# nateraw/pytorchvideo-accelerate

Hardware: AMD Instinct MI355X
Metric: clips/sec (whole node) SlowFast-R50 32x2x224 at 1/2/4/8 MI355X; step-time p50 (higher is better)
Workload: dtype bf16; 1 GPU; model=SlowFast-R50 32x2x224, global_batch=160, per_gpu_batch=160, grad_accum=1, seq_len=32, parallelism=dp1, backend=none, comm=none, forced_sync=False, grad_dtype=fp32, classes=400, hip_graph=False, deterministic=True

## Files before the change

### csrc/kernels/bn_eltwise.hip

```cpp
#include "common.h"
#include <algorithm>

PVA_NS_BEGIN

namespace {

constexpr int NT = 256;

#define ROW_VEC_SETUP(CH)                                  \
  const int vecs = (CH) >> 3;                              \
  const int rpi = NT / vecs;                               \
  const int lr = threadIdx.x / vecs;                       \
  const int c = (threadIdx.x - lr * vecs) << 3;            \
  if (lr >= rpi) return;

__global__ void bn_finalize_kernel(const float* __restrict__ part, int tiles, int C, int64_t count,
                                   const float* __restrict__ gamma, const float* __restrict__ beta,
                                   float* __restrict__ run_mean, float* __restrict__ run_var,
                                   int64_t* __restrict__ nbt, float momentum, float eps,
                                   float* __restrict__ save_mean, float* __restrict__ save_rstd,
                                   float* __restrict__ scale, float* __restrict__ shift) {
  const int c = blockIdx.x;
  double s = 0.0, q = 0.0;
  for (int t = threadIdx.x; t < tiles; t += NT) {
// ... 383 lines not shown
    }
    if constexpr (Y1) {
      float b[8];
      unpack8(*reinterpret_cast<const uint4*>(y1 + m * C + c), b);
#pragma unroll
      for (int e = 0; e < 8; ++e) o[e] = A1[e] * dz[e] + B1[e] * b[e] + C1[e];
      *reinterpret_cast<uint4*>(dy1 + m * C + c) = pack8(o);
    }
    if constexpr (DZ) {
      uint16_t* d = dzout + m * lddz + c;
      if (dz_accum) {
        float q[8];
        unpack8(*reinterpret_cast<const uint4*>(d), q);
#pragma unroll
        for (int e = 0; e < 8; ++e) dz[e] += q[e];
      }
      *reinterpret_cast<uint4*>(d) = pack8(dz);
    }
  }
}

__global__ void stem_pool_fwd_kernel(const uint16_t* __restrict__ y, const float* __restrict__ scale,
                                     const float* __restrict__ shift, uint16_t* __restrict__ out,
                                     uint8_t* __restrict__ arg, uint16_t* __restrict__ ymax, int NT_, int H, int W,
                                     int Ho, int Wo, int C, int ldo) {
  ROW_VEC_SETUP(C);
  float sc[8], sh[8];
#pragma unroll
  for (int e = 0; e < 8; ++e) { sc[e] = scale[c + e]; sh[e] = shift[c + e]; }
  const int Q = NT_ * Ho * Wo;
  for (int q = blockIdx.x * rpi + lr; q < Q; q += gridDim.x * rpi) {
    const int wo = q % Wo;
    const int r = q / Wo;
    const int ho = r % Ho;
    const int nt = r / Ho;
    uint4 v[9];
#pragma unroll
    for (int dh = 0; dh < 3; ++dh)
#pragma unroll
      for (int dw = 0; dw < 3; ++dw) {
        const int h = min(max(ho * 2 - 1 + dh, 0), H - 1), w = min(max(wo * 2 - 1 + dw, 0), W - 1);
        v[dh * 3 + dw] = *reinterpret_cast<const uint4*>(y + (((int64_t)nt * H + h) * W + w) * C + c);
      }
    float best[8], yb[8];
    uint32_t bi[8];
#pragma unroll
    for (int e = 0; e < 8; ++e) { best[e] = -INFINITY; bi[e] = 0; yb[e] = 0.f; }
#pragma unroll
    for (int k = 0; k < 9; ++k) {
      const int h = ho * 2 - 1 + k / 3, w = wo * 2 - 1 + k % 3;
      if ((unsigned)h >= (unsigned)H || (unsigned)w >= (unsigned)W) continue;
      float f[8];
      unpack8(v[k], f);
#pragma unroll
      for (int e = 0; e < 8; ++e) {
        const float a = fmaxf(f[e] * sc[e] + sh[e], 0.f);
        if (a > best[e]) { best[e] = a; bi[e] = (uint32_t)k; yb[e] = f[e]; }
      }
    }
    const int64_t o = (int64_t)q * C + c;
    *reinterpret_cast<uint4*>(out + (int64_t)q * ldo + c) = pack8(best);
    uint2 pk;
    pk.x = bi[0] | (bi[1] << 8) | (bi[2] << 16) | (bi[3] << 24);
    pk.y = bi[4] | (bi[5] << 8) | (bi[6] << 16) | (bi[7] << 24);
    *reinterpret_cast<uint2*>(arg + o) = pk;
    if (ymax) *reinterpret_cast<uint4*>(ymax + o) = pack8(yb);
  }
}

__global__ void stem_pool_bwd_kernel(const uint16_t* __restrict__ dout, int ldd, const uint8_t* __restrict__ arg,
                                     uint16_t* __restrict__ dact, int NT_, int H, int W, int Ho, int Wo, int C) {
  const int vecs = C >> 3;
  const int64_t total = (int64_t)NT_ * H * W * vecs;
  for (int64_t i = blockIdx.x * (int64_t)NT + threadIdx.x; i < total; i += (int64_t)gridDim.x * NT) {
    int64_t r = i;
    const int cv = r % vecs; r /= vecs;
    const int w = r % W; r /= W;
    const int h = r % H; r /= H;
    const int64_t nt = r;
    const int c = cv << 3;
    float acc[8];
#pragma unroll
    for (int e = 0; e < 8; ++e) acc[e] = 0.f;
    const int ho_lo = (h) / 2, ho_hi = min(Ho - 1, (h + 1) / 2);
    const int wo_lo = (w) / 2, wo_hi = min(Wo - 1, (w + 1) / 2);
    for (int ho = ho_lo; ho <= ho_hi; ++ho) {
      const int dh = h - (ho * 2 - 1);
      if (dh < 0 || dh > 2) continue;
      for (int wo = wo_lo; wo <= wo_hi; ++wo) {
        const int dw = w - (wo * 2 - 1);
        if (dw < 0 || dw > 2) continue;
        const int64_t o = (nt * Ho + ho) * Wo + wo;
        const uint2 pk = *reinterpret_cast<const uint2*>(arg + o * C + c);
        float g[8];
        unpack8(*reinterpret_cast<const uint4*>(dout + o * ldd + c), g);
        const uint8_t want = (uint8_t)(dh * 3 + dw);
        uint8_t bi[8] = {(uint8_t)(pk.x), (uint8_t)(pk.x >> 8), (uint8_t)(pk.x >> 16), (uint8_t)(pk.x >> 24),
                         (uint8_t)(pk.y), (uint8_t)(pk.y >> 8), (uint8_t)(pk.y >> 16), (uint8_t)(pk.y >> 24)};
#pragma unroll
        for (int e = 0; e < 8; ++e) if (bi[e] == want) acc[e] += g[e];
      }
    }
    *reinterpret_cast<uint4*>(dact + ((nt * H + h) * W + w) * C + c) = pack8(acc);
  }
}

__global__ void stem_pool_bn_apply_kernel(const uint16_t* __restrict__ dout, int ldd, const uint8_t* __restrict__ arg,
                                          const uint16_t* __restrict__ y, const float* __restrict__ ms,
                                          const float* __restrict__ mh, const float* __restrict__ coef,
                                          uint16_t* __restrict__ dy, int NT_, int H, int W, int Ho, int Wo, int C) {
  ROW_VEC_SETUP(C);
  float A[8], B[8], Cc[8], MS[8], MH[8];
#pragma unroll
  for (int e = 0; e < 8; ++e) {
    A[e] = coef[c + e]; B[e] = coef[C + c + e]; Cc[e] = coef[2 * C + c + e];
    MS[e] = ms[c + e]; MH[e] = mh[c + e];
  }
  const int Q = NT_ * Ho * Wo;
  for (int q = blockIdx.x * rpi + lr; q < Q; q += gridDim.x * rpi) {
    const int wo = q % Wo;
    const int r = q / Wo;
    const int ho = r % Ho;
    const int nt = r / Ho;
    uint2 ag[2][2];
    float g[2][2][8];
#pragma unroll
    for (int i = 0; i < 2; ++i)
#pragma unroll
      for (int j = 0; j < 2; ++j) {
        const bool ok = ho + i < Ho && wo + j < Wo;
        const int64_t o = ((int64_t)nt * Ho + min(ho + i, Ho - 1)) * Wo + min(wo + j, Wo - 1);
        ag[i][j] = *reinterpret_cast<const uint2*>(arg + o * C + c);
        if (!ok) ag[i][j] = make_uint2(0xffffffffu, 0xffffffffu);
        unpack8(*reinterpret_cast<const uint4*>(dout + o * ldd + c), g[i][j]);
      }
#pragma unroll
    for (int a = 0; a < 2; ++a) {
      const int h = 2 * ho + a;
      if (h >= H) continue;
#pragma unroll
      for (int b = 0; b < 2; ++b) {
        const int w = 2 * wo + b;
        if (w >= W) continue;
        const int64_t m = ((int64_t)nt * H + h) * W + w;
        float yv[8], acc[8];
        unpack8(*reinterpret_cast<const uint4*>(y + m * C + c), yv);
#pragma unroll
        for (int e = 0; e < 8; ++e) acc[e] = 0.f;
#pragma unroll
        for (int i = 0; i <= a; ++i)
#pragma unroll
          for (int j = 0; j <= b; ++j) {
            const uint32_t want = (uint32_t)((i ? 0 : a + 1) * 3 + (j ? 0 : b + 1));
            const uint2 pk = ag[i][j];
#pragma unroll
            for (int e = 0; e < 8; ++e) {
              const uint32_t bi = ((e < 4 ? pk.x : pk.y) >> (8 * (e & 3))) & 255u;
              acc[e] += bi == want ? g[i][j][e] : 0.f;
            }
          }
        float o8[8];
#pragma unroll
        for (int e = 0; e < 8; ++e) {
          const float dz = (yv[e] * MS[e] + MH[e]) > 0.f ? acc[e] : 0.f;
          o8[e] = A[e] * dz + B[e] * yv[e] + Cc[e];
        }
        *reinterpret_cast<uint4*>(dy + m * C + c) = pack8(o8);
      }
    }
  }
}

__global__ void avgpool_global_part_kernel(const uint16_t* __restrict__ x, int vol, int C, int S,
                                           float* __restrict__ part) {
  const int n = blockIdx.x / S, sp = blockIdx.x % S;
  const int vecs = C >> 3;
  const int rpi = NT / vecs;
  const int lr = threadIdx.x / vecs;
  const int c = (threadIdx.x - lr * vecs) << 3;
  const int per = (vol + S - 1) / S;
  const int p0 = sp * per, p1 = min(vol, p0 + per);
  float s[8];
#pragma unroll
  for (int e = 0; e < 8; ++e) s[e] = 0.f;
  if (lr < rpi) {
    const uint16_t* base = x + (int64_t)n * vol * C + c;
    int p = p0 + lr;
    for (; p + 3 * rpi < p1; p += 4 * rpi) {
      uint4 q[4];
#pragma unroll
      for (int k = 0; k < 4; ++k) q[k] = *reinterpret_cast<const uint4*>(base + (int64_t)(p + k * rpi) * C);
#pragma unroll
      for (int k = 0; k < 4; ++k) {
        float f[8];
        unpack8(q[k], f);
#pragma unroll
        for (int e = 0; e < 8; ++e) s[e] += f[e];
      }
    }
    for (; p < p1; p += rpi) {
      float f[8];
      unpack8(*reinterpret_cast<const uint4*>(base + (int64_t)p * C), f);
#pragma unroll
      for (int e = 0; e < 8; ++e) s[e] += f[e];
    }
  }
  __shared__ float red[NT * 8];
#pragma unroll
  for (int e = 0; e < 8; ++e) red[threadIdx.x * 8 + e] = s[e];
  __syncthreads();
  for (int i = threadIdx.x; i < C; i += NT) {
    const int v = i >> 3, e = i & 7;
    float t = 0.f;
    for (int k = 0; k < rpi; ++k) t += red[(k * vecs + v) * 8 + e];
    part[((int64_t)n * S + sp) * C + i] = t;
  }
}

__global__ void avgpool_global_final_kernel(const float* __restrict__ part, int S, int C, float inv,
                                            float* __restrict__ out, int ldo, int coff, int N) {
  const int i = blockIdx.x * NT + threadIdx.x;
  if (i >= N * C) return;
  const int n = i / C, c = i % C;
  float t = 0.f;
  for (int k = 0; k < S; ++k) t += part[((int64_t)n * S + k) * C + c];
  out[(int64_t)n * ldo + coff + c] = t * inv;
}

__global__ void avgpool_global_bwd_kernel(const float* __restrict__ dout, int ldo, int coff, int vol, int C,
                                          float inv, uint16_t* __restrict__ dx, int64_t M) {
  ROW_VEC_SETUP(C);
  for (int64_t m = (int64_t)blockIdx.x * rpi + lr; m < M; m += (int64_t)gridDim.x * rpi) {
    const int64_t n = m / vol;
    const float4* src = reinterpret_cast<const float4*>(dout + n * ldo + coff + c);
    const float4 u = src[0], v = src[1];
    float f[8] = {u.x * inv, u.y * inv, u.z * inv, u.w * inv, v.x * inv, v.y * inv, v.z * inv, v.w * inv};
    *reinterpret_cast<uint4*>(dx + m * C + c) = pack8(f);
  }
}

__global__ void avgpool_fwd_kernel(const uint16_t* __restrict__ x, int T, int H, int W, int C, int kt, int kh, int kw,
                                   float* __restrict__ out, int ldo, int coff, int N) {
  const int To = T - kt + 1, Ho = H - kh + 1, Wo = W - kw + 1;
  const int P = To * Ho * Wo;
  const int cg = (C + 63) / 64;
  int b = blockIdx.x;
  const int g = b % cg; b /= cg;
  const int pos = b % P;
  const int n = b / P;
  const int to = pos / (Ho * Wo), ho = (pos / Wo) % Ho, wo = pos % Wo;
  const int lane = threadIdx.x & 63, w = threadIdx.x >> 6;
  const int c = g * 64 + lane;
  const int vol = kt * kh * kw;
  float s = 0.f;
  if (c < C) {
    for (int i = w; i < vol; i += 4) {
      const int a = i / (kh * kw), r = i % (kh * kw), bb = r / kw, d = r % kw;
      s += e2f(x[((((int64_t)n * T + to + a) * H + ho + bb) * W + wo + d) * C + c]);
    }
  }
  __shared__ float red[4][64];
  red[w][lane] = s;
  __syncthreads();
  if (w == 0 && c < C) {
    const float t = red[0][lane] + red[1][lane] + red[2][lane] + red[3][lane];
    out[((int64_t)n * P + pos) * ldo + coff + c] = t / (float)vol;
  }
}

__global__ void avgpool_bwd_kernel(const float* __restrict__ dout, int ldo, int coff, int T, int H, int W, int C,
                                   int kt, int kh, int kw, uint16_t* __restrict__ dx, int N) {
  const int To = T - kt + 1, Ho = H - kh + 1, Wo = W - kw + 1;
  const int64_t total = (int64_t)N * T * H * W * C;
  const float inv = 1.f / (float)(kt * kh * kw);
  for (int64_t i = blockIdx.x * (int64_t)NT + threadIdx.x; i < total; i += (int64_t)gridDim.x * NT) {
    int64_t r = i;
    const int c = r % C; r /= C;
    const int w = r % W; r /= W;
    const int h = r % H; r /= H;
    const int t = r % T; r /= T;
    const int n = (int)r;
    float s = 0.f;
    for (int to = max(0, t - kt + 1); to <= min(To - 1, t); ++to)
      for (int ho = max(0, h - kh + 1); ho <= min(Ho - 1, h); ++ho)
        for (int wo = max(0, w - kw + 1); wo <= min(Wo - 1, w); ++wo)
          s += dout[(((int64_t)n * To + to) * Ho + ho) * Wo * ldo + (int64_t)wo * ldo + coff + c];
    dx[i] = f2e(s * inv);
  }
}

int grid_for(int64_t work) {
  int64_t b = (work + NT - 1) / NT;
  if (b > 8192) b = 8192;
  if (b < 1) b = 1;
  return (int)b;
}

int grid_rows(int64_t M, int C) {
  const int rpi = NT / (C / 8);
  int64_t b = (M + (int64_t)rpi * 4 - 1) / ((int64_t)rpi * 4);
  if (b > 16384) b = 16384;
  if (b < 1) b = 1;
  return (int)b;
}

}

int bn_fin_ranges(int tiles) { return std::min(256, std::max(1, (tiles + FIN_TILES_PER_BLOCK - 1) / FIN_TILES_PER_BLOCK)); }

void bn_finalize_launch(const float* part, int tiles, int C, int64_t count, const float* gamma, const float* beta,
                        float* rm, float* rv, int64_t* nbt, float momentum, float eps, float* smean, float* srstd,
                        float* scale, float* shift, hipStream_t s, double* scratch, unsigned* ctr) {
  if (scratch && ctr) {
    hipLaunchKernelGGL(bn_finalize2_kernel, dim3((C + 63) / 64, bn_fin_ranges(tiles)), dim3(NT), 0, s, part, tiles, C,
                       count, gamma, beta, rm, rv, nbt, momentum, eps, smean, srstd, scale, shift, scratch, ctr);
    return;
  }
  hipLaunchKernelGGL(bn_finalize_kernel, dim3(C), dim3(NT), 0, s, part, tiles, C, count, gamma, beta, rm, rv, nbt,
                     momentum, eps, smean, srstd, scale, shift);
}
// ... 158 lines not shown
```

### csrc/kernels/common.h

```cpp
#pragma once
#include <hip/hip_runtime.h>
#include <stdint.h>

#ifndef PVA_F16
#define PVA_F16 0
#endif
#if PVA_F16
#define PVA_NS pva_f16
typedef _Float16 e16s_t;
#define PVA_MFMA16 __builtin_amdgcn_mfma_f32_16x16x32_f16
#else
#define PVA_NS pva_bf16
typedef __bf16 e16s_t;
#define PVA_MFMA16 __builtin_amdgcn_mfma_f32_16x16x32_bf16
#endif
#define PVA_NS_BEGIN namespace PVA_NS {
#define PVA_NS_END }

typedef uint16_t e16_t;
typedef __attribute__((ext_vector_type(8))) e16s_t ev8_t;
typedef __attribute__((ext_vector_type(4))) float f32x4_t;
typedef __attribute__((ext_vector_type(4))) short s16x4_t;
typedef __attribute__((ext_vector_type(8))) short s16x8_t;
typedef __attribute__((ext_vector_type(2))) float f32x2_t;
typedef __attribute__((ext_vector_type(2))) e16s_t ev2_t;
typedef __attribute__((ext_vector_type(2))) short s16x2_t;

#define PVA_WAVE 64
#define PVA_NXCD 8

#if PVA_F16
__device__ __forceinline__ float e2f(e16_t v) { return (float)__builtin_bit_cast(_Float16, v); }
__device__ __forceinline__ float lo2f(uint32_t w) { return e2f((e16_t)(w & 0xffffu)); }
__device__ __forceinline__ float hi2f(uint32_t w) { return e2f((e16_t)(w >> 16)); }
#else
__device__ __forceinline__ float e2f(e16_t v) { return __uint_as_float(((uint32_t)v) << 16); }
__device__ __forceinline__ float lo2f(uint32_t w) { return __uint_as_float(w << 16); }
__device__ __forceinline__ float hi2f(uint32_t w) { return __uint_as_float(w & 0xffff0000u); }
#endif

__device__ __forceinline__ e16_t f2e(float f) {
  e16s_t b = (e16s_t)f;
  return __builtin_bit_cast(e16_t, b);
}

__device__ __forceinline__ uint32_t cvt_pk_e16(float a, float b) {
  return __builtin_bit_cast(uint32_t, __builtin_convertvector((f32x2_t){a, b}, ev2_t));
}

__device__ __forceinline__ uint32_t pack2(float a, float b) { return cvt_pk_e16(a, b); }

__device__ __forceinline__ void unpack8(const uint4& v, float* f) {
  f[0] = lo2f(v.x); f[1] = hi2f(v.x);
  f[2] = lo2f(v.y); f[3] = hi2f(v.y);
  f[4] = lo2f(v.z); f[5] = hi2f(v.z);
  f[6] = lo2f(v.w); f[7] = hi2f(v.w);
}

__device__ __forceinline__ uint4 pack8(const float* f) {
  return make_uint4(pack2(f[0], f[1]), pack2(f[2], f[3]), pack2(f[4], f[5]), pack2(f[6], f[7]));
}


__device__ __forceinline__ uint4 pack8_fast(const float* f) {
  return make_uint4(cvt_pk_e16(f[0], f[1]), cvt_pk_e16(f[2], f[3]), cvt_pk_e16(f[4], f[5]), cvt_pk_e16(f[6], f[7]));
}

__device__ __forceinline__ uint32_t relu_e16x2(uint32_t w) {
  return __builtin_bit_cast(uint32_t, __builtin_elementwise_max(__builtin_bit_cast(s16x2_t, w), (s16x2_t){0, 0}));
}

__device__ __forceinline__ uint4 relu_e16x8(const uint4& v) {
  return make_uint4(relu_e16x2(v.x), relu_e16x2(v.y), relu_e16x2(v.z), relu_e16x2(v.w));
}

__device__ __forceinline__ uint32_t max_e16x2(uint32_t w, uint32_t floor) {
  return __builtin_bit_cast(uint32_t, __builtin_elementwise_max(__builtin_bit_cast(s16x2_t, w),
                                                                __builtin_bit_cast(s16x2_t, floor)));
}

__device__ __forceinline__ void unpack4(const uint2& v, float* f) {
  f[0] = lo2f(v.x); f[1] = hi2f(v.x);
  f[2] = lo2f(v.y); f[3] = hi2f(v.y);
}

__device__ __forceinline__ uint2 pack4(const float* f) {
  return make_uint2(pack2(f[0], f[1]), pack2(f[2], f[3]));
}

__device__ __forceinline__ int xcd_remap(int orig, int nwg) {
  if (nwg < PVA_NXCD * 2) return orig;
  const int q = nwg / PVA_NXCD, r = nwg % PVA_NXCD;
  const int xcd = orig % PVA_NXCD;
  return (xcd < r ? xcd * (q + 1) : r * (q + 1) + (xcd - r) * q) + orig / PVA_NXCD;
}


template <int CTRL>
__device__ __forceinline__ float dpp_f(float v) {
  return __builtin_bit_cast(float, __builtin_amdgcn_update_dpp(0, __builtin_bit_cast(int, v), CTRL, 0xf, 0xf, false));
}

__device__ __forceinline__ float sum16(float v) {
  v += dpp_f<0xB1>(v);
  v += dpp_f<0x4E>(v);
  v += dpp_f<0x141>(v);
  v += dpp_f<0x140>(v);
  return v;
}

template <int G>
__device__ __forceinline__ float sum_lanes(float v) {
  static_assert(G == 1 || G == 2 || G == 4 || G == 8 || G == 16, "DPP lane groups stay inside a 16-lane row");
  if constexpr (G >= 2) v += dpp_f<0xB1>(v);
  if constexpr (G >= 4) v += dpp_f<0x4E>(v);
  if constexpr (G >= 8) v += dpp_f<0x141>(v);
  if constexpr (G >= 16) v += dpp_f<0x140>(v);
  return v;
}

__device__ __forceinline__ float swap_sum16(float v) {
  const auto r = __builtin_amdgcn_permlane16_swap(__float_as_uint(v), __float_as_uint(v), true, false);
  const unsigned a = r[0], b = r[1];
  return __uint_as_float(a) + __uint_as_float(b);
}
__device__ __forceinline__ float swap_sum32(float v) {
  const auto r = __builtin_amdgcn_permlane32_swap(__float_as_uint(v), __float_as_uint(v), true, false);
  const unsigned a = r[0], b = r[1];
  return __uint_as_float(a) + __uint_as_float(b);
}

template <int S>
__device__ __forceinline__ float wave_sum_stride_c(float v) {
  static_assert(S >= 1 && S <= 64 && (S & (S - 1)) == 0, "stride");
  if constexpr (S <= 1) v += dpp_f<0xB1>(v);
  if constexpr (S <= 2) v += dpp_f<0x4E>(v);
  if constexpr (S <= 4) v += dpp_f<0x124>(v);
  if constexpr (S <= 8) v += dpp_f<0x128>(v);
  if constexpr (S <= 16) v = swap_sum16(v);
  if constexpr (S <= 32) v = swap_sum32(v);
  return v;
}

__device__ __forceinline__ float wave_sum(float v) { return swap_sum32(swap_sum16(sum16(v))); }

__device__ __forceinline__ unsigned swap_partner16(unsigned v) {
  const auto r = __builtin_amdgcn_permlane16_swap(v, v, true, false);
  const unsigned a = r[0], b = r[1];
  return a ^ b ^ v;
}

__device__ __forceinline__ float wave_sum_stride(float v, int S) {
  switch (S) {
    case 1: return wave_sum_stride_c<1>(v);
    case 2: return wave_sum_stride_c<2>(v);
    case 4: return wave_sum_stride_c<4>(v);
    case 8: return wave_sum_stride_c<8>(v);
    case 16: return wave_sum_stride_c<16>(v);
    case 32: return wave_sum_stride_c<32>(v);
    default:
      for (int off = S; off < 64; off <<= 1) v += __shfl_xor(v, off, 64);
      return v;
  }
}

__device__ __forceinline__ float sum_hi4(float v) {
  v += __shfl_xor(v, 16, 64);
  v += __shfl_xor(v, 32, 64);
  return v;
}
```

### csrc/kernels/launchers.h

```cpp
void conv_igemm_launch(const ConvParams& p, int chunk, hipStream_t stream, int cfg);
int conv_cfg_bm(int cfg, int N);
int conv_igemm_ut_legal(const ConvParams& p, int chunk, int bk);
int conv_direct_legal(const ConvParams& p, int chunk);
int conv_pw_legal(const ConvParams& p, int chunk);
int conv_halo_legal(const ConvParams& p, int chunk);
int conv_halo_epi_ok(const ConvParams& p);
int conv_halo64p_legal(const ConvParams& p, int chunk);
void conv_igemm_set_ut(int mode);
int conv_igemm_m_tiles(int M, int N);
int conv_igemm_m_tiles_k(int M, int N, int K, int Cg);
void conv_igemm_set_bk(int bk);
void conv_wgrad_launch(const WgradParams& p, int chunk, hipStream_t stream);
void conv_wgrad_tile(int Cout, int K, int variant, int* bmw, int* bnw);
int wgrad_rt_legal(int Cout, int Cin, int ldd, int ldx, int chunk, int dy_affine);
int wgrad_narrow_legal(int Cout, int Cin, int K);
int wgrad_halo_legal(const WgradParams& p);
int wgrad_box_legal(const WgradParams& p);
void wgrad_box_reduce_launch(const float* slab, float* tmp, float* grad, int splits, int Cout, int taps, int Cin,
                             int Cin_real, float scale, float beta, hipStream_t st);
int wgrad_box_reduce_groups(int splits);
void wgrad_reduce_launch(float* accbuf, float* grad, int splits, int Cout, int taps, int Cin, int Cin_real,
                         float scale, float beta, int slab, hipStream_t stream);
void bn_finalize_launch(const float* part, int tiles, int C, int64_t count, const float* gamma, const float* beta,
                        float* rm, float* rv, int64_t* nbt, float momentum, float eps, float* smean, float* srstd,
                        float* scale, float* shift, hipStream_t s, double* scratch, unsigned* ctr);
int bn_fin_ranges(int tiles);
void bn_eval_affine_launch(int C, const float* gamma, const float* beta, const float* rm, const float* rv, float eps,
                           float* scale, float* shift, hipStream_t s);
void bn_act_launch(const uint16_t* y, int ldy, uint16_t* out, int ldo, const float* scale, const float* shift,
                   int relu, int64_t M, int C, hipStream_t s);
void res_out_launch(const uint16_t* yc, const float* sc, const float* hc, const uint16_t* y1, const float* s1,
                    const float* h1, const uint16_t* x, int ldx, uint16_t* out, int ldo, uint8_t* mask, int64_t M,
                    int C, hipStream_t s);
int bn_bwd_reduce_blocks(int64_t M, int C, int* rows_per_block);
void bn_bwd_reduce_launch(const uint16_t* g, int ldg, int mask_mode, const void* mo, int ldm, const float* ms,
                          const float* mh, const uint16_t* y0, const float* mean0, const float* rstd0,
                          const uint16_t* y1, const float* mean1, const float* rstd1, int64_t M, int C, int blocks,
                          int rows_per_block, float* part, uint16_t* dzout, int lddz, hipStream_t s);
void bn_bwd_finalize_launch(const float* part, int blocks, int C, int64_t count, int which, const float* gamma,
                            const float* mean, const float* rstd, float* dgamma, float* dbeta, float beta_acc,
                            float* coef, hipStream_t s, double* scratch, unsigned* ctr);
void bn_bwd_apply_launch(const uint16_t* g, int ldg, int mask_mode, const void* mo, int ldm, const float* ms,
                         const float* mh, const uint16_t* y0, const float* coef0, uint16_t* dy0, const uint16_t* y1,
                         const float* coef1, uint16_t* dy1, uint16_t* dzout, int lddz, int dz_accum, int64_t M, int C,
                         hipStream_t s);
void stem_pool_fwd_launch(const uint16_t* y, const float* scale, const float* shift, uint16_t* out, uint8_t* arg,
                          uint16_t* ymax, int NT_, int H, int W, int Ho, int Wo, int C, int ldo, hipStream_t s);
void stem_pool_bn_apply_launch(const uint16_t* dout, int ldd, const uint8_t* arg, const uint16_t* y, const float* ms,
                               const float* mh, const float* coef, uint16_t* dy, int NT_, int H, int W, int Ho, int Wo,
                               int C, hipStream_t s);
int avgpool_global_splits(int N, int vol);
void stem_pool_bwd_launch(const uint16_t* dout, int ldd, const uint8_t* arg, uint16_t* dact, int NT_, int H, int W,
                          int Ho, int Wo, int C, hipStream_t s);
void avgpool_fwd_launch(const uint16_t* x, int N, int T, int H, int W, int C, int kt, int kh, int kw, float* out,
                        int ldo, int coff, float* scratch, hipStream_t s);
void avgpool_bwd_launch(const float* dout, int ldo, int coff, int N, int T, int H, int W, int C, int kt, int kh,
                        int kw, uint16_t* dx, hipStream_t s);
void sgd_momentum_launch(float* p, const float* g, float* buf, int64_t n, const float* lr, float momentum, float wd,
                         float gscale, int first, int* found_inf, const int* skip_flag, hipStream_t s);
void nonfinite_check_launch(const float* g, int64_t n, float gscale, int* flag, hipStream_t s);
void pack_weights_launch(const float* master, uint16_t* fwd, uint16_t* dgr, const void* descs, int ntensors,
                         hipStream_t s);
int pack_desc_size();
void video_preprocess_launch(const uint8_t* frames, const int* desc, const int* tidx, int B, int T, int S,
                             const float* mean, const float* std_, uint16_t* out, int s2d, hipStream_t s,
                             const int* slow_of = nullptr, uint16_t* slow_out = nullptr, int Ts = 0);
int stem_tiles(int Ho, int Wo, int N);
void stem_s2d_launch(int mode, const uint16_t* x, const uint16_t* w, uint16_t* y, float* stats, const uint16_t* dy,
                     float* dw, int N, int T, int Hs, int Ws, int Cout, int kt, hipStream_t s, float* slab = nullptr);
bool stem_s2d_supported(int Cout, int kt);
void stem_wgrad_convert_launch(float* acc, float* grad, int Cout, int kt, float beta, hipStream_t s);
void stem_pack_launch(const float* w, uint16_t* out, int Cout, int kt, hipStream_t s);
void synth_frames_launch(uint8_t* out, int64_t n, uint32_t seed, hipStream_t s);

void bnfold_fwd_stats_launch(const uint16_t* Wf, const float* Ga, const float* sslab, int splits, int C, int c,
                             int64_t count, float* T, float* s_out, const float* gamma, const float* beta, float* rm,
                             float* rv, int64_t* nbt, float momentum, float eps, float* smean, float* srstd,
                             float* scale, float* shift, hipStream_t st);
void bnfold_bwd_launch(const float* part, int tiles, const uint16_t* Wf, const uint16_t* Wd, const float* G,
                       const float* T, const float* s, int C, int c, int64_t count, const float* gamma,
                       const float* mean, const float* rstd, float* dgamma, float* dbeta, float* dW, float beta_acc,
                       float* coef, uint16_t* W1t, uint16_t* W2, float* bias, hipStream_t st);
void head_forward_launch(const float* feat, int N, int P, int C, const float* W, const float* b, int K, float p_drop,
                         uint64_t seed, const uint64_t* seedp, float* xm, float* logits, hipStream_t s);
void head_seed_advance_launch(uint64_t* seed, hipStream_t s);
void head_ce_launch(const float* logits, const int64_t* labels, int N, int K, float gscale, float* dlogits,
                    float* row_loss, int* row_correct, float* loss, int64_t* counts, int acc_counts, hipStream_t s);
void head_backward_launch(const float* dlogits, const float* xm, const float* W, int N, int P, int C, int K,
                          float p_drop, uint64_t seed, const uint64_t* seedp, float* dW, float* db, float beta,
                          float* dfeat, float* dlT, float* xmT, float* WT, hipStream_t s);
void head_dropout_mask_launch(int64_t total, float p_drop, uint64_t seed, uint8_t* out, hipStream_t s);
int lateral_bwd_legal(int CO, int Cf, int alpha, int To, int Tf, int kt, int pad);
void lateral_bwd_launch(const uint16_t* g, int ldg, const uint16_t* y, const float* sc, const float* sh,
                        const float* coef, const uint16_t* wd, uint16_t* dy, uint16_t* dx, int ldx, int N, int To,
                        int Tf, int HW, int CO, int Cf, int alpha, hipStream_t s);
int narrow_c_bwd_legal(int CO, int CI);
int narrow_c_bwd_rps(int64_t M, int CO, int splits);
void narrow_c_bwd_launch(const uint16_t* g, int ldg, int mode, const uint8_t* mask, const uint16_t* yc,
                         const float* coef, uint16_t* dz, int lddz, int dz_accum, const uint16_t* yb, const float* sb,
                         const float* hb, const float* mb, const float* rb, const uint16_t* wc, uint16_t* dab, int ldo,
                         int accum, float* slab, float* part, const uint16_t* y1, const float* mc, const float* rc,
                         const float* m1, const float* r1, float* cpart, int form, int64_t M, int CO, int CI, int rps,
                         hipStream_t s);
```

### csrc/kernels/stem_s2d.hip

```cpp
#include "common.h"
#include <stdlib.h>
#include <string.h>
#include <cstdlib>

PVA_NS_BEGIN

namespace {

constexpr int TH = 8, TW = 16;
constexpr int PH = TH + 3, PW = TW + 3;
constexpr int POSB = 32;

struct StemParams {
  const uint16_t* x;
  const uint16_t* w;
  uint16_t* y;
  float* stats;
  const uint16_t* dy;
  float* dw;
  int N, T, Hs, Ws, Cout;
  int To, Ho, Wo;
  int pt;
  int tiles_h, tiles_w;
  int slab;
};

constexpr uint32_t OOB = 0x7ffffff0u;
constexpr int SLOT_BYTES = 448 * 16;

__device__ __forceinline__ void dma16(__amdgpu_buffer_rsrc_t r, char* lds, uint32_t voff) {
#if defined(__HIP_DEVICE_COMPILE__)
  __builtin_amdgcn_raw_ptr_buffer_load_lds(r, (__attribute__((address_space(3))) void*)lds, 16, (int)voff, 0, 0, 0);
#endif
}

__device__ __forceinline__ int pswz(int pos) { return pos ^ ((pos >> 1) & 4); }

template <bool SWZ = false>
__device__ __forceinline__ void dma_patch(__amdgpu_buffer_rsrc_t r, const StemParams& p, int ti, int hs0, int ws0,
                                          char* slot) {
  const int tid = threadIdx.x, w = tid >> 6;
#pragma unroll
  for (int s = 0; s < 2; ++s) {
    if (s == 1 && w == 3) break;
    const int idx = tid + s * 256;
    const int pos = SWZ ? pswz(idx >> 1) : (idx >> 1), half = idx & 1;
    const int r_ = pos / PW, c_ = pos - r_ * PW;
    const int hs = hs0 + r_ - 2, ws = ws0 + c_ - 2;
    const bool ok = pos < PH * PW && ti >= 0 && ti < p.T && (unsigned)hs < (unsigned)p.Hs &&
                    (unsigned)ws < (unsigned)p.Ws;
    const uint32_t vo = ok ? (uint32_t)((((ti * p.Hs + hs) * p.Ws + ws) * 16 + half * 8) * 2) : OOB;
    dma16(r, slot + (w * 64 + s * 256) * 16, vo);
  }
}

__device__ __forceinline__ __amdgpu_buffer_rsrc_t clip_rsrc(const uint16_t* base, uint32_t bytes) {
  return __builtin_amdgcn_make_buffer_rsrc((void*)base, (short)0, (int)bytes, 0x00020000);
}

template <int KT, int COT, bool PERM = false>
__global__ __launch_bounds__(256) __attribute__((amdgpu_waves_per_eu(2))) void stem_fwd_kernel(const StemParams p) {
  constexpr int TAPS = KT * 16;
  constexpr int KSTEPS = TAPS * 16 / 32;
  constexpr int SLOTS = KT + 1;
  extern __shared__ __attribute__((aligned(16))) char smem[];
  float* red = reinterpret_cast<float*>(smem + SLOTS * SLOT_BYTES);

  const int tid = threadIdx.x, lane = tid & 63, w = tid >> 6;
  const int g = lane >> 4, li = lane & 15;
  const int L = xcd_remap(blockIdx.x, gridDim.x);
  int b = L;
  const int tw = b % p.tiles_w; b /= p.tiles_w;
  const int th = b % p.tiles_h;
  const int n = b / p.tiles_h;
  const int ho0 = th * TH, wo0 = tw * TW;

  const __amdgpu_buffer_rsrc_t xr =
      clip_rsrc(p.x + (int64_t)n * p.T * p.Hs * p.Ws * 16, (uint32_t)(p.T * p.Hs * p.Ws * 32));
  ev8_t wa[COT][KSTEPS];
  auto chan = [&](int c, int r) { return PERM ? 32 * (c >> 1) + 8 * (r >> 2) + 4 * (c & 1) + (r & 3) : 16 * c + r; };
#pragma unroll
  for (int c = 0; c < COT; ++c)
#pragma unroll
    for (int ks = 0; ks < KSTEPS; ++ks)
      wa[c][ks] = *reinterpret_cast<const ev8_t*>(p.w + (int64_t)chan(c, li) * (TAPS * 16) + ks * 32 + 8 * g);

  for (int f = 0; f < KT; ++f) dma_patch(xr, p, f - p.pt, ho0, wo0, smem + f * SLOT_BYTES);
  __syncthreads();

  float cs[COT][4], cq[COT][4];
#pragma unroll
  for (int c = 0; c < COT; ++c)
#pragma unroll
    for (int r = 0; r < 4; ++r) { cs[c][r] = 0.f; cq[c][r] = 0.f; }

  const int ww = li;
  const int half = g & 1;
  for (int to = 0; to < p.To; ++to) {
    if (to + 1 < p.To)
      dma_patch(xr, p, to - p.pt + KT, ho0, wo0, smem + ((to + KT) % SLOTS) * SLOT_BYTES);
    f32x4_t acc[2][COT];
#pragma unroll
    for (int q = 0; q < 2; ++q)
#pragma unroll
      for (int c = 0; c < COT; ++c) acc[q][c] = f32x4_t{0.f, 0.f, 0.f, 0.f};
#pragma unroll
    for (int ks = 0; ks < KSTEPS; ++ks) {
      const int tap = 2 * ks + (g >> 1);
      const int dt = tap >> 4, bh = (tap >> 2) & 3, bw = tap & 3;
      const char* slot = smem + ((to + dt) % SLOTS) * SLOT_BYTES;
#pragma unroll
      for (int q = 0; q < 2; ++q) {
        const int hh = 2 * w + q;
        const ev8_t xb = *reinterpret_cast<const ev8_t*>(
            slot + ((hh + bh) * PW + (ww + bw)) * POSB + half * 16);
#pragma unroll
        for (int c = 0; c < COT; ++c)
          acc[q][c] = PVA_MFMA16(wa[c][ks], xb, acc[q][c], 0, 0, 0);
      }
    }
    __syncthreads();
#pragma unroll
    for (int q = 0; q < 2; ++q) {
      const int ho = ho0 + 2 * w + q, wo = wo0 + li;
      const bool valid = ho < p.Ho && wo < p.Wo;
      const int64_t pos = (((int64_t)n * p.To + to) * p.Ho + ho) * p.Wo + wo;
      if constexpr (PERM) {
#pragma unroll
        for (int m = 0; m < COT / 2; ++m) {
          if (valid) {
            float v[8] = {acc[q][2 * m][0], acc[q][2 * m][1], acc[q][2 * m][2], acc[q][2 * m][3],
                          acc[q][2 * m + 1][0], acc[q][2 * m + 1][1], acc[q][2 * m + 1][2], acc[q][2 * m + 1][3]};
            const uint4 pk = pack8(v);
            *reinterpret_cast<uint4*>(p.y + pos * p.Cout + 32 * m + 8 * g) = pk;
            float f[8];
            unpack8(pk, f);
#pragma unroll
            for (int r = 0; r < 4; ++r) {
              cs[2 * m][r] += f[r]; cq[2 * m][r] += f[r] * f[r];
              cs[2 * m + 1][r] += f[4 + r]; cq[2 * m + 1][r] += f[4 + r] * f[4 + r];
            }
          }
        }
        continue;
      }
#pragma unroll
      for (int c = 0; c < COT; ++c) {
        const int co = 16 * c + 4 * g;
        if (valid && co < p.Cout) {
          float v[4] = {acc[q][c][0], acc[q][c][1], acc[q][c][2], acc[q][c][3]};
          const uint2 pk = pack4(v);
          *reinterpret_cast<uint2*>(p.y + pos * p.Cout + co) = pk;
          float f[4];
          unpack4(pk, f);
#pragma unroll
          for (int r = 0; r < 4; ++r) { cs[c][r] += f[r]; cq[c][r] += f[r] * f[r]; }
        }
      }
    }
  }
  constexpr int CT = COT * 16;
#pragma unroll
  for (int c = 0; c < COT; ++c)
#pragma unroll
    for (int r = 0; r < 4; ++r) {
      const float s = sum16(cs[c][r]), q = sum16(cq[c][r]);
      if (li == 0) {
        red[w * 2 * CT + chan(c, 4 * g + r)] = s;
        red[w * 2 * CT + CT + chan(c, 4 * g + r)] = q;
      }
    }
  __syncthreads();
  for (int i = tid; i < p.Cout; i += 256) {
    float s = 0.f, q = 0.f;
#pragma unroll
    for (int k = 0; k < 4; ++k) { s += red[k * 2 * CT + i]; q += red[k * 2 * CT + CT + i]; }
    p.stats[(int64_t)L * 2 * p.Cout + i] = s;
    p.stats[(int64_t)L * 2 * p.Cout + p.Cout + i] = q;
  }
}

__device__ __forceinline__ s16x4_t trr(const char* a) {
  return __builtin_amdgcn_ds_read_tr16_b64_v4i16((__attribute__((address_space(3))) s16x4_t*)(a));
}

__device__ __forceinline__ s16x4_t trr_nw(const char* a) {
  s16x4_t r;
  const uint32_t off = (uint32_t)(uintptr_t)((__attribute__((address_space(3))) const char*)a);
  asm volatile("ds_read_b64_tr_b16 %0, %1" : "=v"(r) : "v"(off));
  return r;
}

template <int N>
__device__ __forceinline__ void lgkm_tie(s16x4_t& a, s16x4_t& b, s16x4_t& c, s16x4_t& d) {
  asm volatile("s_waitcnt lgkmcnt(%4)" : "+v"(a), "+v"(b), "+v"(c), "+v"(d) : "n"(N));
}

__device__ __forceinline__ ev8_t frag8(s16x4_t lo, s16x4_t hi) {
  s16x8_t v = {lo[0], lo[1], lo[2], lo[3], hi[0], hi[1], hi[2], hi[3]};
  return __builtin_bit_cast(ev8_t, v);
}

template <int KT, int COT, bool AR = false>
__global__ __launch_bounds__(256) void stem_wgrad_kernel(const StemParams p) {
  constexpr int TAPS = KT * 16;
  constexpr int TPW = TAPS / 4;
  constexpr int SLOTS = KT + 1;
  constexpr int COP = COT * 16;
  constexpr int DYB = TH * TW * COP * 2;
  constexpr int DYC = TH * TW * COP / 8 / 256;
  extern __shared__ __attribute__((aligned(16))) char smem[];
  char* dyt = smem + SLOTS * SLOT_BYTES;

  const int tid = threadIdx.x, lane = tid & 63, w = tid >> 6;
  const int g = lane >> 4, li = lane & 15;
  const int L = xcd_remap(blockIdx.x, gridDim.x);
  int b = L;
  const int tw = b % p.tiles_w; b /= p.tiles_w;
  const int th = b % p.tiles_h;
  const int n = b / p.tiles_h;
  const int ho0 = th * TH, wo0 = tw * TW;
  const __amdgpu_buffer_rsrc_t xr =
      clip_rsrc(p.x + (int64_t)n * p.T * p.Hs * p.Ws * 16, (uint32_t)(p.T * p.Hs * p.Ws * 32));
  const __amdgpu_buffer_rsrc_t yr = clip_rsrc(p.dy + (int64_t)n * p.To * p.Ho * p.Wo * p.Cout,
                                              (uint32_t)(p.To * p.Ho * p.Wo * p.Cout * 2));
  auto dma_dy = [&](int to, char* buf) {
#pragma unroll
    for (int k = 0; k < DYC; ++k) {
      const int idx = tid + k * 256;
      const int pos = idx / (COP / 8), ch = (idx % (COP / 8)) * 8;
      const int ho = ho0 + pos / TW, wo = wo0 + pos % TW;
      const bool ok = ho < p.Ho && wo < p.Wo && ch < p.Cout;
      const uint32_t vo = ok ? (uint32_t)((((to * p.Ho + ho) * p.Wo + wo) * p.Cout + ch) * 2) : OOB;
      dma16(yr, buf + (k * 256 + w * 64) * 16, vo);
    }
  };

  f32x4_t acc[COT][TPW];
#pragma unroll
  for (int c = 0; c < COT; ++c)
#pragma unroll
    for (int t = 0; t < TPW; ++t) acc[c][t] = f32x4_t{0.f, 0.f, 0.f, 0.f};

  for (int f = 0; f < KT; ++f) dma_patch(xr, p, f - p.pt, ho0, wo0, smem + f * SLOT_BYTES);
  dma_dy(0, dyt);
  __syncthreads();
  const int rq = li >> 2, cb = (li & 3) * 8;
  for (int to = 0; to < p.To; ++to) {
    const char* dcur = dyt + (to & 1) * DYB;
    if (to + 1 < p.To) {
      dma_patch(xr, p, to - p.pt + KT, ho0, wo0, smem + ((to + KT) % SLOTS) * SLOT_BYTES);
      dma_dy(to + 1, dyt + ((to + 1) & 1) * DYB);
    }
    if constexpr (AR) {
      constexpr int KS = TH * TW / 32, NR = COT + TPW;
      static_assert(NR % 2 == 0, "ties go by 4 halves");
      s16x4_t R[2][NR][2];
      auto issue = [&](int kstep, s16x4_t (&Rk)[NR][2]) {
        const int hh = 2 * kstep + (g >> 1), wq = 8 * (g & 1) + rq;
#pragma unroll
        for (int c = 0; c < COT; ++c) {
          const char* base = dcur + (hh * TW + wq) * COP * 2 + c * 32 + cb;
          Rk[c][0] = trr_nw(base);
          Rk[c][1] = trr_nw(base + 4 * COP * 2);
        }
#pragma unroll
        for (int t = 0; t < TPW; ++t) {
          const int tap = w * TPW + t;
          const int dt = tap >> 4, bh = (tap >> 2) & 3, bw = tap & 3;
          const char* base = smem + ((to + dt) % SLOTS) * SLOT_BYTES + ((hh + bh) * PW + (wq + bw)) * POSB + cb;
          Rk[COT + t][0] = trr_nw(base);
          Rk[COT + t][1] = trr_nw(base + 4 * POSB);
        }
      };
      issue(0, R[0]);
#pragma unroll
      for (int kstep = 0; kstep < KS; ++kstep) {
        s16x4_t(&Rk)[NR][2] = R[kstep & 1];
        if (kstep + 1 < KS) {
          issue(kstep + 1, R[(kstep + 1) & 1]);
#pragma unroll
          for (int i = 0; i < NR; i += 2) lgkm_tie<(2 * NR < 15 ? 2 * NR : 15)>(Rk[i][0], Rk[i][1], Rk[i + 1][0], Rk[i + 1][1]);
        } else {
#pragma unroll
          for (int i = 0; i < NR; i += 2) lgkm_tie<0>(Rk[i][0], Rk[i][1], Rk[i + 1][0], Rk[i + 1][1]);
        }
#pragma unroll
        for (int t = 0; t < TPW; ++t) {
          const ev8_t xb = frag8(Rk[COT + t][0], Rk[COT + t][1]);
#pragma unroll
          for (int c = 0; c < COT; ++c) acc[c][t] = PVA_MFMA16(frag8(Rk[c][0], Rk[c][1]), xb, acc[c][t], 0, 0, 0);
        }
      }
      __syncthreads();
      continue;
    }
#pragma unroll
    for (int kstep = 0; kstep < TH * TW / 32; ++kstep) {
      const int hh = 2 * kstep + (g >> 1);
      const int wq = 8 * (g & 1) + rq;
      ev8_t a[COT];
#pragma unroll
      for (int c = 0; c < COT; ++c) {
        const char* base = dcur + (hh * TW + wq) * COP * 2 + c * 32 + cb;
        s16x4_t lo = trr(base), hi = trr(base + 4 * COP * 2);
        s16x8_t v = {lo[0], lo[1], lo[2], lo[3], hi[0], hi[1], hi[2], hi[3]};
        a[c] = __builtin_bit_cast(ev8_t, v);
      }
#pragma unroll
      for (int t = 0; t < TPW; ++t) {
        const int tap = w * TPW + t;
        const int dt = tap >> 4, bh = (tap >> 2) & 3, bw = tap & 3;
        const char* slot = smem + ((to + dt) % SLOTS) * SLOT_BYTES;
        const char* base = slot + ((hh + bh) * PW + (wq + bw)) * POSB + cb;
        s16x4_t lo = trr(base), hi = trr(base + 4 * POSB);
        s16x8_t v = {lo[0], lo[1], lo[2], lo[3], hi[0], hi[1], hi[2], hi[3]};
        const ev8_t xb = __builtin_bit_cast(ev8_t, v);
#pragma unroll
        for (int c = 0; c < COT; ++c)
          acc[c][t] = PVA_MFMA16(a[c], xb, acc[c][t], 0, 0, 0);
      }
    }
    __syncthreads();
  }
#pragma unroll
  for (int c = 0; c < COT; ++c)
#pragma unroll
    for (int t = 0; t < TPW; ++t) {
      const int tap = w * TPW + t;
#pragma unroll
      for (int r = 0; r < 4; ++r) {
        const int co = 16 * c + 4 * g + r;
        if (co < p.Cout) {
          const int64_t o = (int64_t)co * TAPS * 16 + tap * 16 + li;
          if (p.slab) p.dw[(int64_t)blockIdx.x * p.slab + o] = acc[c][t][r];
          else atomicAdd(p.dw + o, acc[c][t][r]);
        }
      }
    }
}

__device__ __forceinline__ ev8_t ld_frag(const uint16_t* p, bool ok) {
  const uint4 u = ok ? *reinterpret_cast<const uint4*>(p) : make_uint4(0, 0, 0, 0);
  return __builtin_bit_cast(ev8_t, u);
}

template <int KT>
__global__ __launch_bounds__(256) __attribute__((amdgpu_waves_per_eu(2))) void stem_fwd_pair_kernel(const StemParams p) {
  constexpr int TAPS = KT * 16;
  constexpr int J = KT + 1;
  constexpr int KS = 8;
  constexpr int SLOTS = J + 2;
  extern __shared__ __attribute__((aligned(16))) char smem[];
  float* red = reinterpret_cast<float*>(smem + SLOTS * SLOT_BYTES);

  const int tid = threadIdx.x, lane = tid & 63, w = tid >> 6;
  const int g = lane >> 4, li = lane & 15;
  const int L = xcd_remap(blockIdx.x, gridDim.x);
  int b = L;
  const int tw = b % p.tiles_w; b /= p.tiles_w;
  const int th = b % p.tiles_h;
  const int n = b / p.tiles_h;
  const int ho0 = th * TH, wo0 = tw * TW;
  const __amdgpu_buffer_rsrc_t xr =
      clip_rsrc(p.x + (int64_t)n * p.T * p.Hs * p.Ws * 16, (uint32_t)(p.T * p.Hs * p.Ws * 32));

  for (int f = 0; f < J; ++f) dma_patch(xr, p, f - p.pt, ho0, wo0, smem + f * SLOT_BYTES);

  ev8_t wa[J][KS];
#pragma unroll
  for (int j = 0; j < J; ++j) {
    const int dt = li < 8 ? j : j - 1;
    const bool ok = dt >= 0 && dt < KT;
#pragma unroll
    for (int ks = 0; ks < KS; ++ks)
      wa[j][ks] = ld_frag(p.w + (int64_t)(li & 7) * (TAPS * 16) + (ok ? dt : 0) * 256 + ks * 32 + 8 * g, ok);
  }
  __syncthreads();

  float cs[4] = {0.f, 0.f, 0.f, 0.f}, cq[4] = {0.f, 0.f, 0.f, 0.f};
  const int half = g & 1;
  const int co0 = 4 * (g & 1);
  for (int t0 = 0; t0 < p.To; t0 += 2) {
    if (t0 + 2 < p.To) {
      const int tn = t0 - p.pt + J;
      dma_patch(xr, p, tn, ho0, wo0, smem + ((t0 + J) % SLOTS) * SLOT_BYTES);
      dma_patch(xr, p, tn + 1, ho0, wo0, smem + ((t0 + J + 1) % SLOTS) * SLOT_BYTES);
    }
    f32x4_t acc[2] = {f32x4_t{0.f, 0.f, 0.f, 0.f}, f32x4_t{0.f, 0.f, 0.f, 0.f}};
#pragma unroll
    for (int j = 0; j < J; ++j) {
      const char* slot = smem + ((t0 + j) % SLOTS) * SLOT_BYTES;
#pragma unroll
      for (int ks = 0; ks < KS; ++ks) {
        const int tap = 2 * ks + (g >> 1);
        const int bh = tap >> 2, bw = tap & 3;
#pragma unroll
        for (int q = 0; q < 2; ++q) {
          const ev8_t xb = *reinterpret_cast<const ev8_t*>(
              slot + ((2 * w + q + bh) * PW + (li + bw)) * POSB + half * 16);
          acc[q] = PVA_MFMA16(wa[j][ks], xb, acc[q], 0, 0, 0);
        }
      }
    }
    __syncthreads();
    const int to = t0 + (g >> 1);
#pragma unroll
    for (int q = 0; q < 2; ++q) {
      const int ho = ho0 + 2 * w + q, wo = wo0 + li;
      if (ho < p.Ho && wo < p.Wo && to < p.To) {
        const int64_t pos = (((int64_t)n * p.To + to) * p.Ho + ho) * p.Wo + wo;
        float v[4] = {acc[q][0], acc[q][1], acc[q][2], acc[q][3]};
        const uint2 pk = pack4(v);
        *reinterpret_cast<uint2*>(p.y + pos * 8 + co0) = pk;
        float f[4];
        unpack4(pk, f);
#pragma unroll
        for (int r = 0; r < 4; ++r) { cs[r] += f[r]; cq[r] += f[r] * f[r]; }
      }
    }
  }
#pragma unroll
  for (int r = 0; r < 4; ++r) {
    float s = sum16(cs[r]), q = sum16(cq[r]);
    s += __shfl_xor(s, 32, 64);
    q += __shfl_xor(q, 32, 64);
    if (li == 0 && g < 2) {
      red[w * 16 + 4 * g + r] = s;
      red[w * 16 + 8 + 4 * g + r] = q;
    }
  }
  __syncthreads();
  if (tid < 8) {
    float s = 0.f, q = 0.f;
#pragma unroll
    for (int k = 0; k < 4; ++k) { s += red[k * 16 + tid]; q += red[k * 16 + 8 + tid]; }
    p.stats[(int64_t)L * 16 + tid] = s;
    p.stats[(int64_t)L * 16 + 8 + tid] = q;
  }
}

template <int KT, bool ROLL, bool AR = false>
__global__ __launch_bounds__(256) __attribute__((amdgpu_waves_per_eu(2))) void stem_wgrad_pair_kernel(const StemParams p) {
  constexpr int TAPS = KT * 16;
  constexpr int J = KT + 1;
  constexpr int SLOTS = J + 2;
  constexpr int DYB = TH * TW * 16 * 2;
  extern __shared__ __attribute__((aligned(16))) char smem[];
  char* dyt = smem + SLOTS * SLOT_BYTES;

  const int tid = threadIdx.x, lane = tid & 63, w = tid >> 6;
  const int g = lane >> 4, li = lane & 15;
  const int L = xcd_remap(blockIdx.x, gridDim.x);
  int b = L;
  const int tw = b % p.tiles_w; b /= p.tiles_w;
  const int th = b % p.tiles_h;
  const int n = b / p.tiles_h;
  const int ho0 = th * TH, wo0 = tw * TW;
  const __amdgpu_buffer_rsrc_t xr =
      clip_rsrc(p.x + (int64_t)n * p.T * p.Hs * p.Ws * 16, (uint32_t)(p.T * p.Hs * p.Ws * 32));
  const __amdgpu_buffer_rsrc_t yr =
      clip_rsrc(p.dy + (int64_t)n * p.To * p.Ho * p.Wo * 8, (uint32_t)(p.To * p.Ho * p.Wo * 16));
  const int dpos = pswz(tid >> 1), dfh = tid & 1;
  const int dho = ho0 + dpos / TW, dwo = wo0 + dpos % TW;
  const bool dok = dho < p.Ho && dwo < p.Wo;
  auto dma_dy = [&](int t0, char* buf) {
    const int to = t0 + dfh;
    const uint32_t vo = dok && to < p.To ? (uint32_t)((((to * p.Ho + dho) * p.Wo + dwo) * 8) * 2) : OOB;
    dma16(yr, buf + w * 64 * 16, vo);
  };

  f32x4_t acc[J][4];
#pragma unroll
  for (int j = 0; j < J; ++j)
#pragma unroll
    for (int s = 0; s < 4; ++s) acc[j][s] = f32x4_t{0.f, 0.f, 0.f, 0.f};

  for (int f = 0; f < J; ++f) dma_patch<true>(xr, p, f - p.pt, ho0, wo0, smem + f * SLOT_BYTES);
  dma_dy(0, dyt);
  __syncthreads();
  const int rq = li >> 2, cb = (li & 3) * 8;
  for (int t0 = 0; t0 < p.To; t0 += 2) {
    const char* dcur = dyt + ((t0 >> 1) & 1) * DYB;
    if (t0 + 2 < p.To) {
      const int tn = t0 - p.pt + J;
      dma_patch<true>(xr, p, tn, ho0, wo0, smem + ((t0 + J) % SLOTS) * SLOT_BYTES);
      dma_patch<true>(xr, p, tn + 1, ho0, wo0, smem + ((t0 + J + 1) % SLOTS) * SLOT_BYTES);
      dma_dy(t0 + 2, dyt + (((t0 >> 1) + 1) & 1) * DYB);
    }
    if constexpr (ROLL && AR) {
      constexpr int KS = TH * TW / 32;
      const int h0 = g >> 1, wq = 8 * (g & 1) + rq;
      ev8_t af[KS];
      {
        s16x4_t al[KS], ah[KS];
#pragma unroll
        for (int kstep = 0; kstep < KS; ++kstep) {
          const int dp = (2 * kstep + h0) * TW + wq;
          al[kstep] = trr_nw(dcur + pswz(dp) * 32 + cb);
          ah[kstep] = trr_nw(dcur + pswz(dp + 4) * 32 + cb);
        }
        lgkm_tie<0>(al[0], ah[0], al[1], ah[1]);
        lgkm_tie<0>(al[2], ah[2], al[3], ah[3]);
#pragma unroll
        for (int kstep = 0; kstep < KS; ++kstep) af[kstep] = frag8(al[kstep], ah[kstep]);
      }
#pragma unroll
      for (int j = 0; j < J; ++j) {
        const char* slot = smem + ((t0 + j) % SLOTS) * SLOT_BYTES;
        s16x4_t F[KS + 1][4];
        auto issue = [&](int m) {
#pragma unroll
          for (int e = 0; e < 2; ++e) {
            const int ip = (2 * m + h0 + e) * PW + wq + w;
            F[m][2 * e] = trr_nw(slot + pswz(ip) * POSB + cb);
            F[m][2 * e + 1] = trr_nw(slot + pswz(ip + 4) * POSB + cb);
          }
        };
        issue(0);
        issue(1);
#pragma unroll
        for (int kstep = 0; kstep < KS; ++kstep) {
          if (kstep + 2 <= KS) {
            issue(kstep + 2);
            if (kstep == 0) lgkm_tie<4>(F[0][0], F[0][1], F[0][2], F[0][3]);
            lgkm_tie<4>(F[kstep + 1][0], F[kstep + 1][1], F[kstep + 1][2], F[kstep + 1][3]);
          } else {
            lgkm_tie<0>(F[kstep + 1][0], F[kstep + 1][1], F[kstep + 1][2], F[kstep + 1][3]);
          }
          acc[j][0] = PVA_MFMA16(af[kstep], frag8(F[kstep][0], F[kstep][1]), acc[j][0], 0, 0, 0);
          acc[j][1] = PVA_MFMA16(af[kstep], frag8(F[kstep][2], F[kstep][3]), acc[j][1], 0, 0, 0);
          acc[j][2] = PVA_MFMA16(af[kstep], frag8(F[kstep + 1][0], F[kstep + 1][1]), acc[j][2], 0, 0, 0);
          acc[j][3] = PVA_MFMA16(af[kstep], frag8(F[kstep + 1][2], F[kstep + 1][3]), acc[j][3], 0, 0, 0);
        }
      }
      __syncthreads();
      continue;
    }
    if constexpr (ROLL) {
      constexpr int KS = TH * TW / 32;
      const int h0 = g >> 1, wq = 8 * (g & 1) + rq;
      ev8_t af[KS];
#pragma unroll
      for (int kstep = 0; kstep < KS; ++kstep) {
        const int dp = (2 * kstep + h0) * TW + wq;
        s16x4_t lo = trr(dcur + pswz(dp) * 32 + cb), hi = trr(dcur + pswz(dp + 4) * 32 + cb);
        s16x8_t v = {lo[0], lo[1], lo[2], lo[3], hi[0], hi[1], hi[2], hi[3]};
        af[kstep] = __builtin_bit_cast(ev8_t, v);
      }
#pragma unroll
      for (int j = 0; j < J; ++j) {
        const char* slot = smem + ((t0 + j) % SLOTS) * SLOT_BYTES;
        auto frag = [&](int row) {
          const int ip = row * PW + wq + w;
          s16x4_t lo = trr(slot + pswz(ip) * POSB + cb), hi = trr(slot + pswz(ip + 4) * POSB + cb);
          s16x8_t v = {lo[0], lo[1], lo[2], lo[3], hi[0], hi[1], hi[2], hi[3]};
          return __builtin_bit_cast(ev8_t, v);
        };
        ev8_t fe = frag(h0), fo = frag(h0 + 1);
#pragma unroll
        for (int kstep = 0; kstep < KS; ++kstep) {
          const int hh = 2 * kstep + h0;
          const ev8_t fe2 = frag(hh + 2), fo2 = frag(hh + 3);
          acc[j][0] = PVA_MFMA16(af[kstep], fe, acc[j][0], 0, 0, 0);
          acc[j][1] = PVA_MFMA16(af[kstep], fo, acc[j][1], 0, 0, 0);
          acc[j][2] = PVA_MFMA16(af[kstep], fe2, acc[j][2], 0, 0, 0);
          acc[j][3] = PVA_MFMA16(af[kstep], fo2, acc[j][3], 0, 0, 0);
          fe = fe2;
          fo = fo2;
        }
      }
      __syncthreads();
      continue;
    }
#pragma unroll
    for (int kstep = 0; kstep < TH * TW / 32; ++kstep) {
      const int hh = 2 * kstep + (g >> 1);
      const int wq = 8 * (g & 1) + rq;
      ev8_t a;
      {
        const int dp = hh * TW + wq;
        s16x4_t lo = trr(dcur + pswz(dp) * 32 + cb), hi = trr(dcur + pswz(dp + 4) * 32 + cb);
        s16x8_t v = {lo[0], lo[1], lo[2], lo[3], hi[0], hi[1], hi[2], hi[3]};
        a = __builtin_bit_cast(ev8_t, v);
      }
#pragma unroll
      for (int j = 0; j < J; ++j) {
        const char* slot = smem + ((t0 + j) % SLOTS) * SLOT_BYTES;
#pragma unroll
        for (int s = 0; s < 4; ++s) {
          const int ip = (hh + w) * PW + (wq + s);
          s16x4_t lo = trr(slot + pswz(ip) * POSB + cb), hi = trr(slot + pswz(ip + 4) * POSB + cb);
          s16x8_t v = {lo[0], lo[1], lo[2], lo[3], hi[0], hi[1], hi[2], hi[3]};
          acc[j][s] = PVA_MFMA16(a, __builtin_bit_cast(ev8_t, v), acc[j][s], 0, 0, 0);
        }
      }
    }
    __syncthreads();
  }
#pragma unroll
  for (int dt = 0; dt < KT; ++dt)
#pragma unroll
    for (int s = 0; s < 4; ++s)
#pragma unroll
      for (int r = 0; r < 4; ++r) {
        float v = g < 2 ? acc[dt][s][r] : acc[dt + 1][s][r];
        v += __shfl_xor(v, 32, 64);
        const int tap = ROLL ? 4 * s + w : 4 * w + s;
        if (g < 2) {
          const int64_t o = (int64_t)(4 * g + r) * TAPS * 16 + (dt * 16 + tap) * 16 + li;
          if (p.slab) p.dw[(int64_t)blockIdx.x * p.slab + o] = v;
          else atomicAdd(p.dw + o, v);
        }
      }
}

__global__ __launch_bounds__(256) void stem_slab_reduce_kernel(const float* slab, int nslab, int n, float* acc) {
  const int i = blockIdx.x * blockDim.x + threadIdx.x;
  if (i >= n) return;
  float v = acc[i];
  for (int k = 0; k < nslab; ++k) v += slab[(int64_t)k * n + i];
  acc[i] = v;
}

__global__ void stem_wgrad_convert_kernel(float* __restrict__ acc, float* __restrict__ grad, int Cout, int kt,
                                          float beta) {
  const int total = Cout * 3 * kt * 49;
  for (int o = blockIdx.x * blockDim.x + threadIdx.x; o < total; o += gridDim.x * blockDim.x) {
    int r = o;
    const int kw = r % 7; r /= 7;
    const int kh = r % 7; r /= 7;
    const int dt = r % kt; r /= kt;
    const int c = r % 3;
    const int co = r / 3;
    const int bh = (kh + 1) >> 1, sy = (kh + 1) & 1, bw = (kw + 1) >> 1, sx = (kw + 1) & 1;
    const int a = co * kt * 256 + ((dt * 4 + bh) * 4 + bw) * 16 + (sy * 2 + sx) * 4 + c;
    grad[o] = (beta == 0.f ? 0.f : beta * grad[o]) + acc[a];
  }
}

__global__ void zero_kernel(float* p, int n) {
  for (int i = blockIdx.x * blockDim.x + threadIdx.x; i < n; i += gridDim.x * blockDim.x) p[i] = 0.f;
}

__global__ void stem_pack_kernel(const float* __restrict__ w, uint16_t* __restrict__ out, int Cout, int Cpad, int kt) {
  const int K = kt * 256;
  const int total = Cpad * K;
  for (int i = blockIdx.x * blockDim.x + threadIdx.x; i < total; i += gridDim.x * blockDim.x) {
    const int co = i / K;
    int k = i % K;
    const int ch = k % 16, tap = k / 16;
    const int c = ch % 4, sx = (ch / 4) & 1, sy = ch / 8;
    const int bw = tap % 4, bh = (tap / 4) % 4, dt = tap / 16;
    const int kh = 2 * bh + sy - 1, kw = 2 * bw + sx - 1;
    float v = 0.f;
    if (co < Cout && c < 3 && kh >= 0 && kh < 7 && kw >= 0 && kw < 7)
      v = w[(((co * 3 + c) * kt + dt) * 7 + kh) * 7 + kw];
    out[i] = f2e(v);
  }
}

template <int KT, int COT, bool PERM = false>
void launch_fwd(const StemParams& p, hipStream_t s) {
  const size_t lds = (KT + 1) * SLOT_BYTES + 4 * 2 * COT * 16 * 4;
  hipLaunchKernelGGL((stem_fwd_kernel<KT, COT, PERM>), dim3(p.N * p.tiles_h * p.tiles_w), dim3(256), lds, s, p);
}

template <int KT, int COT, bool AR = false>
void launch_wgrad(const StemParams& p, hipStream_t s) {
  const size_t lds = (KT + 1) * SLOT_BYTES + 2 * TH * TW * COT * 16 * 2;
  hipLaunchKernelGGL((stem_wgrad_kernel<KT, COT, AR>), dim3(p.N * p.tiles_h * p.tiles_w), dim3(256), lds, s, p);
}

template <int KT>
void launch_fwd_pair(const StemParams& p, hipStream_t s) {
  const size_t lds = (KT + 3) * SLOT_BYTES + 4 * 16 * 4;
  hipLaunchKernelGGL((stem_fwd_pair_kernel<KT>), dim3(p.N * p.tiles_h * p.tiles_w), dim3(256), lds, s, p);
}

template <int KT, bool ROLL, bool AR = false>
void launch_wgrad_pair(const StemParams& p, hipStream_t s) {
  const size_t lds = (KT + 3) * SLOT_BYTES + 2 * TH * TW * 16 * 2;
  hipLaunchKernelGGL((stem_wgrad_pair_kernel<KT, ROLL, AR>), dim3(p.N * p.tiles_h * p.tiles_w), dim3(256), lds, s, p);
}

}

int stem_tiles(int Ho, int Wo, int N) { return N * ((Ho + TH - 1) / TH) * ((Wo + TW - 1) / TW); }

static int stem_arm(const char* name) {
  const char* e = getenv("PVA_ARMS");
  if (e == nullptr) return 1;
  const size_t n = strlen(name);
  for (const char* p = strstr(e, name); p != nullptr; p = strstr(p + 1, name)) {
    const bool start = p == e || p[-1] == ',' || p[-1] == ' ';
    if (start && p[n] == '=') return atoi(p + n + 1);
  }
  return 1;
}
static bool stem_pair_enabled() { return stem_arm("stem_pair") != 0; }
static bool stem_perm_enabled() { return stem_arm("stem_perm") != 0; }
static bool stem_roll_enabled() { return stem_arm("stem_roll") != 0; }
static bool stem_async_enabled() { return stem_arm("stem_async") != 0; }

void stem_s2d_launch(int mode, const uint16_t* x, const uint16_t* w, uint16_t* y, float* stats, const uint16_t* dy,
                     float* dw, int N, int T, int Hs, int Ws, int Cout, int kt, hipStream_t s, float* slab) {
  StemParams p{};
  p.x = x; p.w = w; p.y = y; p.stats = stats; p.dy = dy; p.dw = slab != nullptr ? slab : dw;
  p.slab = slab != nullptr ? Cout * kt * 256 : 0;
  p.N = N; p.T = T; p.Hs = Hs; p.Ws = Ws; p.Cout = Cout;
  p.To = T; p.Ho = Hs; p.Wo = Ws; p.pt = kt / 2;
  p.tiles_h = (Hs + TH - 1) / TH; p.tiles_w = (Ws + TW - 1) / TW;
  const bool pair = stem_pair_enabled() && kt == 5 && Cout == 8;
  if (mode == 0) {
    if (pair) launch_fwd_pair<5>(p, s);
    else if (kt == 5 && Cout <= 16) launch_fwd<5, 1>(p, s);
    else if (kt == 1 && Cout == 64 && stem_perm_enabled()) launch_fwd<1, 4, true>(p, s);
    else if (kt == 1 && Cout <= 64) launch_fwd<1, 4>(p, s);
  } else {
    if (pair && stem_roll_enabled() && stem_async_enabled()) launch_wgrad_pair<5, true, true>(p, s);
    else if (pair && stem_roll_enabled()) launch_wgrad_pair<5, true>(p, s);
    else if (pair) launch_wgrad_pair<5, false>(p, s);
    else if (kt == 5 && Cout <= 16) launch_wgrad<5, 1>(p, s);
    else if (kt == 1 && Cout <= 64 && stem_async_enabled()) launch_wgrad<1, 4, true>(p, s);
    else if (kt == 1 && Cout <= 64) launch_wgrad<1, 4>(p, s);
    if (slab != nullptr) {
      const int n = Cout * kt * 256, nslab = p.N * p.tiles_h * p.tiles_w;
      hipLaunchKernelGGL(stem_slab_reduce_kernel, dim3((n + 255) / 256), dim3(256), 0, s, slab, nslab, n, dw);
    }
  }
}

bool stem_s2d_supported(int Cout, int kt) { return (kt == 5 && Cout <= 16) || (kt == 1 && Cout <= 64); }

void stem_wgrad_convert_launch(float* acc, float* grad, int Cout, int kt, float beta, hipStream_t s) {
  const int total = Cout * 3 * kt * 49;
  hipLaunchKernelGGL(stem_wgrad_convert_kernel, dim3((total + 255) / 256), dim3(256), 0, s, acc, grad, Cout, kt, beta);
  const int n = Cout * kt * 256;
  hipLaunchKernelGGL(zero_kernel, dim3((n + 255) / 256), dim3(256), 0, s, acc, n);
}

void stem_pack_launch(const float* w, uint16_t* out, int Cout, int kt, hipStream_t s) {
  const int Cpad = (Cout + 15) / 16 * 16;
  const int total = Cpad * kt * 256;
  hipLaunchKernelGGL(stem_pack_kernel, dim3((total + 255) / 256), dim3(256), 0, s, w, out, Cout, Cpad, kt);
}

PVA_NS_END
```

### csrc/runtime/bindings.cpp

```cpp
#include <torch/extension.h>
#include <ATen/hip/HIPContext.h>
#include <hip/hip_runtime.h>
#include <rocprofiler-sdk-roctx/roctx.h>

#include "../kernels/conv_params.h"
#include <cstddef>

static_assert(offsetof(ConvParams, bws) - offsetof(ConvParams, M) == 38 * sizeof(int),
              "ConvParams integer block must be contiguous (filled from a 39-int geometry vector)");

namespace pva_bf16 {
#include "../kernels/launchers.h"
}
namespace pva_f16 {
#include "../kernels/launchers.h"
}
void register_clip_reader(pybind11::module& m);
void register_rccl(pybind11::module& m);
void register_fp32(pybind11::module& m);

namespace {

using OptT = c10::optional<at::Tensor>;

// ... 285 lines not shown
}

void bn_bwd_reduce(const at::Tensor& g, int64_t ldg, int64_t mask_mode, const OptT& mo, int64_t ldm, const OptT& ms,
                   const OptT& mh, const OptT& y0, const OptT& mean0, const OptT& rstd0,
                   const OptT& y1, const OptT& mean1, const OptT& rstd1, int64_t M, int64_t C, int64_t blocks,
                   int64_t rpb, const at::Tensor& part, const OptT& dzout, int64_t lddz) {
  const bool h = kind16(g);
  TORCH_CHECK(C % 8 == 0 && C <= 2048, "bn_bwd_reduce channel constraint");
  TORCH_CHECK(!dzout.has_value() || (lddz % 8 == 0 && dzout->size(0) >= M), "bn_bwd_reduce: dz output layout");
  TORCH_CHECK(!y0.has_value() || (mean0.has_value() && rstd0.has_value()), "y0 needs mean0/rstd0");
  TORCH_CHECK(mask_mode != 2 || y0.has_value(), "mask mode 2 reads y0");
  KSEL(h, bn_bwd_reduce_launch)(bfp(g), (int)ldg, (int)mask_mode, mask_ptr(mask_mode, mo), (int)ldm, f32o(ms), f32o(mh), bfo(y0), f32o(mean0),
                       f32o(rstd0), bfo(y1), f32o(mean1), f32o(rstd1), M, (int)C, (int)blocks, (int)rpb, f32(part),
                       bfom(dzout), (int)lddz, cur_stream());
}

void bn_bwd_finalize(const at::Tensor& part, int64_t blocks, int64_t C, int64_t count, int64_t which,
                     const at::Tensor& gamma, const at::Tensor& mean, const at::Tensor& rstd, const OptT& dgamma,
                     const OptT& dbeta, double beta_acc, const at::Tensor& coef, const OptT& fin) {
  double* scr = nullptr;
  unsigned* ctr = nullptr;
  fin_buffers(fin, C, &scr, &ctr);
  pva_bf16::bn_bwd_finalize_launch(f32(part), (int)blocks, (int)C, count, (int)which, f32(gamma), f32(mean), f32(rstd),
                         f32o(dgamma), f32o(dbeta), (float)beta_acc, f32(coef), cur_stream(), scr, ctr);
}

void bn_bwd_apply(const at::Tensor& g, int64_t ldg, int64_t mask_mode, const OptT& mo, int64_t ldm, const OptT& ms,
                  const OptT& mh, const OptT& y0, const OptT& coef0, const OptT& dy0,
                  const OptT& y1, const OptT& coef1, const OptT& dy1, const OptT& dzout, int64_t lddz,
                  int64_t dz_accum, int64_t M, int64_t C) {
  const bool h = kind16(g);
  TORCH_CHECK(y0.has_value() == coef0.has_value() && y0.has_value() == dy0.has_value(), "y0/coef0/dy0 go together");
  TORCH_CHECK(mask_mode != 2 || y0.has_value(), "mask mode 2 reads y0");
  KSEL(h, bn_bwd_apply_launch)(bfp(g), (int)ldg, (int)mask_mode, mask_ptr(mask_mode, mo), (int)ldm, f32o(ms), f32o(mh), bfo(y0), f32o(coef0),
                      bfom(dy0), bfo(y1), f32o(coef1), bfom(dy1), bfom(dzout), (int)lddz, (int)dz_accum, M, (int)C,
                      cur_stream());
}

void stem_pool_fwd(const at::Tensor& y, const at::Tensor& scale, const at::Tensor& shift, const at::Tensor& out,
                   int64_t ldo, const at::Tensor& arg, int64_t NT_, int64_t H, int64_t W, int64_t Ho, int64_t Wo,
                   int64_t C, const OptT& ymax) {
  const bool h = kind16(y);
  TORCH_CHECK(C % 8 == 0 && ldo % 8 == 0, "stem pool: channels / row stride must be multiples of 8");
  TORCH_CHECK(arg.numel() >= NT_ * Ho * Wo * C, "stem pool: argmax buffer too small");
  TORCH_CHECK(!ymax.has_value() || ymax->numel() >= NT_ * Ho * Wo * C, "stem pool: ymax buffer too small");
  TORCH_CHECK(NT_ * H * W < ((int64_t)1 << 31) && C <= 2048, "stem pool: position count exceeds int32");
  TORCH_CHECK(Ho == (H - 1) / 2 + 1 && Wo == (W - 1) / 2 + 1, "stem pool: 3x3/s2/p1 output dims");
  KSEL(h, stem_pool_fwd_launch)(bfp(y), f32(scale), f32(shift), bfpm(out), arg.data_ptr<uint8_t>(), bfom(ymax), (int)NT_,
                       (int)H, (int)W, (int)Ho, (int)Wo, (int)C, (int)ldo, cur_stream());
}

void stem_pool_bn_apply(const at::Tensor& dout, int64_t ldd, const at::Tensor& arg, const at::Tensor& y,
                        const at::Tensor& ms, const at::Tensor& mh, const at::Tensor& coef, const at::Tensor& dy,
                        int64_t NT_, int64_t H, int64_t W, int64_t Ho, int64_t Wo, int64_t C) {
  const bool h = kind16(dout);
  TORCH_CHECK(C % 8 == 0 && ldd % 8 == 0 && C <= 2048, "stem pool bwd: channel layout");
  TORCH_CHECK(NT_ * H * W < ((int64_t)1 << 31), "stem pool bwd: position count exceeds int32");
  TORCH_CHECK(y.numel() >= NT_ * H * W * C && dy.numel() >= NT_ * H * W * C, "stem pool bwd: y/dy too small");
  TORCH_CHECK(arg.numel() >= NT_ * Ho * Wo * C && dout.dim() == 2 && dout.size(0) >= NT_ * Ho * Wo &&
              dout.size(1) >= C && dout.stride(0) == ldd, "stem pool bwd: pooled buffers / row stride");
  TORCH_CHECK(Ho == (H - 1) / 2 + 1 && Wo == (W - 1) / 2 + 1, "stem pool bwd: 3x3/s2/p1 output dims");
  KSEL(h, stem_pool_bn_apply_launch)(bfp(dout), (int)ldd, arg.data_ptr<uint8_t>(), bfp(y), f32(ms), f32(mh), f32(coef), bfpm(dy),
                            (int)NT_, (int)H, (int)W, (int)Ho, (int)Wo, (int)C, cur_stream());
}

void stem_pool_bwd(const at::Tensor& dout, int64_t ldd, const at::Tensor& arg, const at::Tensor& dact, int64_t NT_,
                   int64_t H, int64_t W, int64_t Ho, int64_t Wo, int64_t C) {
  const bool h = kind16(dout);
  KSEL(h, stem_pool_bwd_launch)(bfp(dout), (int)ldd, arg.data_ptr<uint8_t>(), bfpm(dact), (int)NT_, (int)H, (int)W, (int)Ho,
                       (int)Wo, (int)C, cur_stream());
}

void avgpool_fwd(const at::Tensor& x, std::vector<int64_t> dims, std::vector<int64_t> k, const at::Tensor& out,
                 int64_t ldo, int64_t coff) {
  const bool h = kind16(x);
  const int N = (int)dims[0], T = (int)dims[1], H = (int)dims[2], W = (int)dims[3], C = (int)dims[4];
  at::Tensor scratch;
  if (k[0] == T && k[1] == H && k[2] == W)
    scratch = at::empty({(int64_t)N * KSEL(h, avgpool_global_splits)(N, T * H * W) * C}, out.options());
  KSEL(h, avgpool_fwd_launch)(bfp(x), N, T, H, W, C, (int)k[0], (int)k[1], (int)k[2], f32(out), (int)ldo, (int)coff,
                     scratch.defined() ? scratch.data_ptr<float>() : nullptr, cur_stream());
}

void avgpool_bwd(const at::Tensor& dout, int64_t ldo, int64_t coff, std::vector<int64_t> dims, std::vector<int64_t> k,
                 const at::Tensor& dx) {
  const bool h = kind16(dx);
  KSEL(h, avgpool_bwd_launch)(f32(dout), (int)ldo, (int)coff, (int)dims[0], (int)dims[1], (int)dims[2], (int)dims[3],
                     (int)dims[4], (int)k[0], (int)k[1], (int)k[2], bfpm(dx), cur_stream());
}

void sgd_momentum(const at::Tensor& p, const at::Tensor& g, const at::Tensor& buf, const at::Tensor& lr,
                  double momentum, double wd, double gscale, int64_t first, const OptT& found_inf,
                  const OptT& skip_if) {
  TORCH_CHECK(p.numel() == g.numel() && p.numel() == buf.numel(), "sgd buffers must match");
  int* fi = found_inf.has_value() ? found_inf->data_ptr<int>() : nullptr;
  const int* sk = skip_if.has_value() ? skip_if->data_ptr<int>() : nullptr;
  pva_bf16::sgd_momentum_launch(f32(p), f32(g), f32(buf), p.numel(), f32(lr), (float)momentum, (float)wd, (float)gscale,
                      (int)first, fi, sk, cur_stream());
}

void nonfinite_check(const at::Tensor& g, double gscale, const at::Tensor& flag) {
  TORCH_CHECK(flag.scalar_type() == at::kInt, "flag must be int32");
  pva_bf16::nonfinite_check_launch(f32(g), g.numel(), (float)gscale, flag.data_ptr<int>(), cur_stream());
}

void pack_weights(const at::Tensor& master, const at::Tensor& fwd, const at::Tensor& dgr, const at::Tensor& descs,
                  int64_t ntensors) {
  const bool h = kind16(fwd);
  KSEL(h, pack_weights_launch)(f32(master), bfpm(fwd), bfpm(dgr), descs.data_ptr(), (int)ntensors, cur_stream());
}

void video_preprocess(const at::Tensor& frames, const at::Tensor& desc, const at::Tensor& tidx, int64_t T, int64_t S,
                      std::vector<double> mean, std::vector<double> std_, const at::Tensor& out, bool s2d,
                      const OptT& slow_of, const OptT& slow_out, int64_t Ts) {
  const bool h = kind16(out);
  TORCH_CHECK(!s2d || S % 2 == 0, "space-to-depth output needs an even crop");
  TORCH_CHECK(frames.scalar_type() == at::kByte, "frames must be uint8");
  TORCH_CHECK(desc.dim() == 2 && desc.size(1) == 10 && desc.scalar_type() == at::kInt, "desc [B,10] int32");
  TORCH_CHECK(tidx.dim() == 2 && tidx.size(1) == T && tidx.scalar_type() == at::kInt, "tidx [B,T] int32");
  TORCH_CHECK(out.numel() >= desc.size(0) * T * S * S * 4, "output too small");
  const float m[3] = {(float)mean[0], (float)mean[1], (float)mean[2]};
  const float s[3] = {(float)std_[0], (float)std_[1], (float)std_[2]};
  TORCH_CHECK(slow_of.has_value() == slow_out.has_value(), "slow_of and slow_out go together");
  if (slow_of.has_value()) {
    TORCH_CHECK(slow_of->scalar_type() == at::kInt && slow_of->numel() == T, "slow_of [T] int32");
    TORCH_CHECK(slow_out->numel() >= desc.size(0) * Ts * S * S * 4 && kind16(*slow_out) == h, "slow output size / type");
  }
  KSEL(h, video_preprocess_launch)(frames.data_ptr<uint8_t>(), desc.data_ptr<int>(), tidx.data_ptr<int>(), (int)desc.size(0),
                          (int)T, (int)S, m, s, bfpm(out), s2d ? 1 : 0, cur_stream(),
                          slow_of.has_value() ? slow_of->data_ptr<int>() : nullptr, bfom(slow_out), (int)Ts);
}

void stem_fwd(const at::Tensor& x, const at::Tensor& wpack, const at::Tensor& y, const at::Tensor& stats,
              std::vector<int64_t> dims, int64_t Cout, int64_t kt) {
  const bool h = kind16(x);
  TORCH_CHECK(KSEL(h, stem_s2d_supported)((int)Cout, (int)kt), "unsupported stem");
  TORCH_CHECK(x.size(1) == 16 && x.is_contiguous(), "stem input must be dense s2d [M,16]");
  const int N = dims[0], T = dims[1], Hs = dims[2], Ws = dims[3];
  TORCH_CHECK(stats.numel() >= (int64_t)KSEL(h, stem_tiles)(Hs, Ws, N) * 2 * Cout, "stats too small");
  KSEL(h, stem_s2d_launch)(0, bfp(x), bfp(wpack), bfpm(y), f32(stats), nullptr, nullptr, N, T, Hs, Ws, (int)Cout, (int)kt,
                  cur_stream(), nullptr);
}

void stem_wgrad(const at::Tensor& x, const at::Tensor& dy, const at::Tensor& acc, std::vector<int64_t> dims,
                int64_t Cout, int64_t kt, const OptT& slab) {
  const bool h = kind16(x);
  TORCH_CHECK(KSEL(h, stem_s2d_supported)((int)Cout, (int)kt), "unsupported stem");
  TORCH_CHECK(acc.numel() >= Cout * kt * 256, "accumulator too small");
  const int N = dims[0], T = dims[1], Hs = dims[2], Ws = dims[3];
  TORCH_CHECK(!slab.has_value() || slab->numel() >= (int64_t)KSEL(h, stem_tiles)(Hs, Ws, N) * Cout * kt * 256,
              "stem slab too small");
  KSEL(h, stem_s2d_launch)(1, bfp(x), nullptr, nullptr, nullptr, bfp(dy), f32(acc), N, T, Hs, Ws, (int)Cout, (int)kt,
                  cur_stream(), f32o(slab));
}

inline const uint64_t* seed_ptr(const OptT& t) {
  if (!t.has_value()) return nullptr;
  TORCH_CHECK(t->scalar_type() == at::kLong && t->numel() >= 1 && t->is_cuda(), "device seed must be int64 [1]");
  return reinterpret_cast<const uint64_t*>(t->data_ptr<int64_t>());
}

void head_forward(const at::Tensor& feat, const at::Tensor& W, const OptT& b, double p_drop, int64_t seed,
                  const at::Tensor& xm, const at::Tensor& logits, const OptT& seed_dev) {
  TORCH_CHECK(feat.dim() == 3 && feat.is_contiguous(), "feat must be [N][P][C] contiguous");
  const int N = feat.size(0), P = feat.size(1), C = feat.size(2), K = W.size(0);
  TORCH_CHECK(W.dim() == 2 && W.size(1) == C && W.is_contiguous(), "W must be [K][C]");
  TORCH_CHECK(xm.numel() >= (int64_t)N * C && logits.numel() >= (int64_t)N * K, "head outputs too small");
  TORCH_CHECK(p_drop >= 0.0 && p_drop < 1.0, "dropout probability must be in [0, 1)");
  if (N == 0) return;
  pva_bf16::head_forward_launch(f32(feat), N, P, C, f32(W), f32o(b), K, (float)p_drop, (uint64_t)seed, seed_ptr(seed_dev),
                      f32(xm), f32(logits), cur_stream());
}

void head_ce(const at::Tensor& logits, const OptT& labels, double gscale, const OptT& dlogits, const OptT& loss,
             const OptT& counts, int64_t acc_counts, const at::Tensor& row_loss, const at::Tensor& row_correct) {
  const int N = logits.size(0), K = logits.size(1);
  TORCH_CHECK(!labels.has_value() || (labels->scalar_type() == at::kLong && labels->numel() == N), "labels int64 [N]");
  TORCH_CHECK(!counts.has_value() || (counts->scalar_type() == at::kLong && counts->numel() >= 2), "counts int64 [2]");
  TORCH_CHECK(row_correct.scalar_type() == at::kInt && row_correct.numel() >= N && row_loss.numel() >= N, "row scratch");
  if (N == 0) return;
  pva_bf16::head_ce_launch(f32(logits), labels.has_value() ? labels->data_ptr<int64_t>() : nullptr, N, K, (float)gscale,
                 f32o(dlogits), f32(row_loss), row_correct.data_ptr<int>(), f32o(loss),
                 counts.has_value() ? counts->data_ptr<int64_t>() : nullptr, (int)acc_counts, cur_stream());
}

void head_backward(const at::Tensor& dlogits, const at::Tensor& xm, const at::Tensor& W, int64_t P, double p_drop,
                   int64_t seed, const at::Tensor& dW, const OptT& db, double beta, const OptT& dfeat,
                   const at::Tensor& scratch, const OptT& seed_dev) {
  const int N = dlogits.size(0), K = dlogits.size(1), C = W.size(1);
  TORCH_CHECK(xm.numel() >= (int64_t)N * C && dW.numel() == (int64_t)K * C, "head backward shapes");
  TORCH_CHECK(!dfeat.has_value() || dfeat->numel() >= (int64_t)N * P * C, "dfeat too small");
  TORCH_CHECK(scratch.numel() >= (int64_t)K * N + (int64_t)C * N + (int64_t)C * K, "head scratch too small");
  if (N == 0) return;
  float* sc = f32(scratch);
  pva_bf16::head_backward_launch(f32(dlogits), f32(xm), f32(W), N, (int)P, C, K, (float)p_drop, (uint64_t)seed,
                       seed_ptr(seed_dev), f32(dW),
                       f32o(db), (float)beta, f32o(dfeat), sc, sc + (int64_t)K * N, sc + (int64_t)K * N + (int64_t)C * N,
                       cur_stream());
}

void bnfold_fwd_stats(const at::Tensor& Wf, const at::Tensor& Ga, const at::Tensor& sslab, int64_t splits, int64_t C,
                      int64_t c, int64_t count, const at::Tensor& T, const at::Tensor& s_out, const at::Tensor& gamma,
                      const at::Tensor& beta, const OptT& rm, const OptT& rv, const OptT& nbt, double momentum,
                      double eps, const at::Tensor& smean, const at::Tensor& srstd, const at::Tensor& scale,
                      const at::Tensor& shift) {
  const bool h = kind16(Wf);
  TORCH_CHECK(c % 8 == 0 && c <= 2048 && Wf.numel() >= C * c && Ga.numel() >= c * c && T.numel() >= C * c,
              "bnfold_fwd_stats shapes");
  TORCH_CHECK(sslab.numel() >= splits * c && s_out.numel() >= c, "bnfold colsum shapes");
  int64_t* nb = nbt.has_value() ? nbt->data_ptr<int64_t>() : nullptr;
  KSEL(h, bnfold_fwd_stats_launch)(bfp(Wf), f32(Ga), f32(sslab), (int)splits, (int)C, (int)c, count, f32(T), f32(s_out),
                          f32(gamma), f32(beta), f32o(rm), f32o(rv), nb, (float)momentum, (float)eps, f32(smean),
                          f32(srstd), f32(scale), f32(shift), cur_stream());
}

void bnfold_bwd(const at::Tensor& part, int64_t tiles, const at::Tensor& Wf, const at::Tensor& Wd, const at::Tensor& G,
                const at::Tensor& T, const at::Tensor& s, int64_t C, int64_t c, int64_t count, const at::Tensor& gamma,
                const at::Tensor& mean, const at::Tensor& rstd, const OptT& dgamma, const OptT& dbeta,
                const at::Tensor& dW, double beta_acc, const at::Tensor& coef, const at::Tensor& W1t,
                const at::Tensor& W2, const at::Tensor& bias) {
  const bool h = kind16(Wf);
  TORCH_CHECK(c % 8 == 0 && Wf.numel() >= C * c && Wd.numel() >= C * c && G.numel() >= C * c && T.numel() >= C * c &&
              dW.numel() == C * c && coef.numel() >= 4 * C && W1t.numel() >= C * c && W2.numel() >= c * c &&
              bias.numel() >= 2 * c && part.numel() >= tiles * 3 * C, "bnfold_bwd shapes");
  KSEL(h, bnfold_bwd_launch)(f32(part), (int)tiles, bfp(Wf), bfp(Wd), f32(G), f32(T), f32(s), (int)C, (int)c, count,
                    f32(gamma), f32(mean), f32(rstd), f32o(dgamma), f32o(dbeta), f32(dW), (float)beta_acc, f32(coef),
                    bfpm(W1t), bfpm(W2), f32(bias), cur_stream());
}

void head_seed_advance(const at::Tensor& seed_dev) {
  TORCH_CHECK(seed_dev.scalar_type() == at::kLong && seed_dev.numel() >= 1 && seed_dev.is_cuda(), "int64 [1] seed");
  pva_bf16::head_seed_advance_launch(reinterpret_cast<uint64_t*>(seed_dev.data_ptr<int64_t>()), cur_stream());
}

void head_dropout_mask(const at::Tensor& out, double p_drop, int64_t seed) {
  TORCH_CHECK(out.scalar_type() == at::kByte, "mask must be uint8");
  pva_bf16::head_dropout_mask_launch(out.numel(), (float)p_drop, (uint64_t)seed, out.data_ptr<uint8_t>(), cur_stream());
}

void narrow_c_bwd(const at::Tensor& g, int64_t ldg, int64_t mode, const OptT& mask, const OptT& yc,
                  const at::Tensor& coef, const OptT& dz, int64_t lddz, int64_t dz_accum, const at::Tensor& yb,
                  const OptT& sb, const OptT& hb, const OptT& mb, const OptT& rb, const at::Tensor& wc,
                  const OptT& dab, int64_t ldo, int64_t accum, const OptT& slab, const OptT& part, int64_t M,
                  int64_t CO, int64_t CI, int64_t rps, int64_t form, const OptT& y1, const OptT& mc, const OptT& rc,
                  const OptT& m1, const OptT& r1, const OptT& cpart) {
  const bool h = kind16(g);
  TORCH_CHECK(pva_bf16::narrow_c_bwd_legal((int)CO, (int)CI), "narrow_c_bwd: unsupported channels");
  TORCH_CHECK(mode == 0 || (mode == 3 && mask.has_value()), "narrow_c_bwd: mask mode 0 or 3 (bits)");
  TORCH_CHECK(form >= 0 && form <= 2, "narrow_c_bwd: form 0, 1 or 2");
  TORCH_CHECK(form != 0 || (yc.has_value() && yc->numel() >= M * CO), "narrow_c_bwd: form 0 reads yc");
  TORCH_CHECK(yb.numel() >= M * CI && wc.numel() >= CO * CI, "narrow_c_bwd: tensor sizes");
  TORCH_CHECK(ldg % 8 == 0 && (!dz.has_value() || lddz % 8 == 0) && ldo % 2 == 0, "narrow_c_bwd: aligned rows");
  const bool bn = sb.has_value();
  TORCH_CHECK(bn == (hb.has_value() && mb.has_value() && rb.has_value()), "narrow_c_bwd: BN_b scale/shift/mean/rstd");
  const int64_t splits = (M + rps - 1) / rps;
  if (form == 2) {
    TORCH_CHECK(bn && mc.has_value() && rc.has_value() && cpart.has_value() && cpart->numel() >= splits * 3 * CO,
                "narrow_c_bwd reduce: BN_b affine, BN_c mean/rstd and the partial-sum buffer");
    TORCH_CHECK(!y1.has_value() || (m1.has_value() && r1.has_value() && y1->numel() >= M * CO),
                "narrow_c_bwd reduce: branch1 needs its mean / rstd");
  } else {
    TORCH_CHECK(dab.has_value() && dab->numel() >= (M - 1) * ldo + CI && slab.has_value() &&
                slab->numel() >= splits * CO * CI, "narrow_c_bwd: dab / slab sizes");
    TORCH_CHECK(!bn || (part.has_value() && part->numel() >= splits * 3 * CI), "narrow_c_bwd: BN_b partial sums");
    TORCH_CHECK(!(bn && accum), "narrow_c_bwd: the BN_b-masked input gradient is written, not accumulated");
  }
  KSEL(h, narrow_c_bwd_launch)(bfp(g), (int)ldg, (int)mode, mask.has_value() ? mask->data_ptr<uint8_t>() : nullptr,
                               bfo(yc), f32(coef), bfom(dz), (int)lddz, (int)dz_accum, bfp(yb), f32o(sb), f32o(hb),
                               f32o(mb), f32o(rb), bfp(wc), bfom(dab), (int)ldo, (int)accum, f32o(slab), f32o(part),
                               bfo(y1), f32o(mc), f32o(rc), f32o(m1), f32o(r1), f32o(cpart), (int)form, M, (int)CO,
                               (int)CI, (int)rps, cur_stream());
}

void lateral_bwd(const at::Tensor& g, int64_t ldg, const at::Tensor& y, const at::Tensor& sc, const at::Tensor& sh,
                 const at::Tensor& coef, const at::Tensor& wd, const OptT& dy, const at::Tensor& dx, int64_t ldx,
                 int64_t N, int64_t To, int64_t Tf, int64_t HW, int64_t CO, int64_t Cf, int64_t alpha) {
  const bool h = kind16(g);
  TORCH_CHECK(pva_bf16::lateral_bwd_legal((int)CO, (int)Cf, (int)alpha, (int)To, (int)Tf, 7, 3),
              "lateral_bwd: unsupported geometry");
  TORCH_CHECK(ldg % 8 == 0 && ldx % 8 == 0 && ldg >= CO && ldx >= Cf, "lateral_bwd: 16-B aligned rows");
  TORCH_CHECK(y.numel() >= N * To * HW * CO && g.dim() == 2 && g.size(0) >= N * To * HW && g.size(1) >= CO &&
              g.stride(0) == ldg, "lateral_bwd: slow sizes");
  TORCH_CHECK(dx.dim() == 2 && dx.size(0) >= N * Tf * HW && dx.size(1) >= Cf && dx.stride(0) == ldx &&
              wd.numel() >= Cf * 7 * CO, "lateral_bwd: fast sizes");
  TORCH_CHECK(!dy.has_value() || dy->numel() >= N * To * HW * CO, "lateral_bwd: dy size");
  TORCH_CHECK(To * HW * ldg < (1LL << 30) && Tf * HW * ldx < (1LL << 30), "lateral_bwd: per-clip 32-bit offsets");
  KSEL(h, lateral_bwd_launch)(bfp(g), (int)ldg, bfp(y), f32(sc), f32(sh), f32(coef), bfp(wd), bfom(dy), bfpm(dx),
                              (int)ldx, (int)N, (int)To, (int)Tf, (int)HW, (int)CO, (int)Cf, (int)alpha, cur_stream());
}

void synth_frames(const at::Tensor& out, int64_t seed) {
  pva_bf16::synth_frames_launch(out.data_ptr<uint8_t>(), out.numel(), (uint32_t)seed, cur_stream());
}

}

extern "C" const char pva_build_id_str[];

PYBIND11_MODULE(_C, m) {
  m.doc() = "gfx950 HIP kernels for pytorchvideo_accelerate_amd";
  m.def("build_id", []() { return std::string(pva_build_id_str + 13); });
  m.def("range_push", [](const std::string& s) { return (int64_t)roctxRangePushA(s.c_str()); });
  m.def("range_pop", []() { return (int64_t)roctxRangePop(); });
  m.def("trace_mark", [](const std::string& s) { roctxMarkA(s.c_str()); });
  m.def("conv_igemm", &conv_igemm, py::arg("x"), py::arg("w"), py::arg("y"), py::arg("stats"), py::arg("scale"),
        py::arg("shift"), py::arg("affine"), py::arg("accum"), py::arg("g"), py::arg("chunk"), py::arg("cfg") = -1,
        py::arg("bias") = py::none(), py::arg("nostore") = 0);
  m.def("conv_igemm_fres", &conv_igemm_fres);
  m.def("bnfold_fwd_stats", &bnfold_fwd_stats);
  m.def("bnfold_bwd", &bnfold_bwd);
  m.def("conv_cfg_bm", [](int64_t cfg, int64_t N) { return (int64_t)pva_bf16::conv_cfg_bm((int)cfg, (int)N); });
  m.def("conv_ut_legal", [](std::vector<int64_t> g, int64_t chunk, int64_t bk) {
    ConvParams q{};
    int* f = &q.M;
    for (int i = 0; i < 39 && i < (int)g.size(); ++i) f[i] = (int)g[i];
    return (int64_t)pva_bf16::conv_igemm_ut_legal(q, (int)chunk, (int)bk);
  });
  m.def("wgrad_halo_legal", [](std::vector<int64_t> g, int64_t variant, int64_t affine) {
    TORCH_CHECK(g.size() == 23, "wgrad geometry must have 23 entries");
    WgradParams p{};
    p.P = g[0]; p.Cout = g[1]; p.K = g[2]; p.Cin = g[3]; p.ldd = g[4]; p.ldx = g[5];
    p.Ti = g[6]; p.Hi = g[7]; p.Wi = g[8]; p.To = g[9]; p.Ho = g[10]; p.Wo = g[11];
    p.kt = g[12]; p.kh = g[13]; p.kw = g[14]; p.st = g[15]; p.sh = g[16]; p.sw = g[17];
    p.pt = g[18]; p.ph = g[19]; p.pw = g[20]; p.splits = g[21]; p.p_per_split = g[22];
    p.variant = (int)variant; p.affine = (int)affine;
    return (int64_t)pva_bf16::wgrad_halo_legal(p);
  });
  m.def("conv_pw_legal", [](std::vector<int64_t> g, int64_t chunk) {
    ConvParams q{};
    int* f = &q.M;
    for (int i = 0; i < 39 && i < (int)g.size(); ++i) f[i] = (int)g[i];
    auto dim_ok = [](int R, int as, int ao, int dir, int n, int G) {
      const int lo = ao + (dir < 0 ? -(n - 1) : 0);
      const int hi = (R - 1) * as + ao + (dir > 0 ? (n - 1) : 0);
      return n == 0 || (lo >= 0 && hi < G);
    };
    q.check = (dim_ok(q.Rt, q.ast, q.aot, q.dir, q.nt, q.Gt) && dim_ok(q.Rh, q.ash, q.aoh, q.dir, q.nh, q.Gh) &&
               dim_ok(q.Rw, q.asw, q.aow, q.dir, q.nw, q.Gw)) ? 0 : 1;
    return (int64_t)pva_bf16::conv_pw_legal(q, (int)chunk);
  });
  m.def("wgrad_box_reduce", &wgrad_box_reduce);
  m.def("box_reduce_groups", [](int64_t splits) { return (int64_t)pva_bf16::wgrad_box_reduce_groups((int)splits); });
  m.def("wgrad_box_legal", [](std::vector<int64_t> g) {
    WgradParams q{};
    q.P = g[0]; q.Cout = g[1]; q.K = g[2]; q.Cin = g[3]; q.ldd = g[4]; q.ldx = g[5];
    q.Ti = g[6]; q.Hi = g[7]; q.Wi = g[8]; q.To = g[9]; q.Ho = g[10]; q.Wo = g[11];
    q.kt = g[12]; q.kh = g[13]; q.kw = g[14]; q.st = g[15]; q.sh = g[16]; q.sw = g[17];
    q.pt = g[18]; q.ph = g[19]; q.pw = g[20];
    return (int64_t)pva_bf16::wgrad_box_legal(q);
  });
  m.def("conv_halo64p_legal", [](std::vector<int64_t> g, int64_t chunk) {
    ConvParams q{};
    int* f = &q.M;
    for (int i = 0; i < 39 && i < (int)g.size(); ++i) f[i] = (int)g[i];
    return (int64_t)pva_bf16::conv_halo64p_legal(q, (int)chunk);
  });
  m.def("conv_halo_legal", [](std::vector<int64_t> g, int64_t chunk) {
    ConvParams q{};
    int* f = &q.M;
    for (int i = 0; i < 39 && i < (int)g.size(); ++i) f[i] = (int)g[i];
    return (int64_t)pva_bf16::conv_halo_legal(q, (int)chunk);
  });
  m.def("conv_direct_legal", [](std::vector<int64_t> g, int64_t chunk) {
    ConvParams q{};
    int* f = &q.M;
    for (int i = 0; i < 39 && i < (int)g.size(); ++i) f[i] = (int)g[i];
    return (int64_t)pva_bf16::conv_direct_legal(q, (int)chunk);
  });
  m.def("conv_igemm_epi", &conv_igemm_epi, py::arg("x"), py::arg("w"), py::arg("y"), py::arg("accum"), py::arg("g"),
        py::arg("chunk"), py::arg("res"), py::arg("ldr"), py::arg("mask"), py::arg("y0"), py::arg("mean0"),
        py::arg("rstd0"), py::arg("y1"), py::arg("mean1"), py::arg("rstd1"), py::arg("part"),
        py::arg("msc") = py::none(), py::arg("msh") = py::none(), py::arg("cfg") = -1, py::arg("bias") = py::none());
  m.def("conv_m_tiles", &conv_m_tiles, py::arg("M"), py::arg("N"), py::arg("K") = 0, py::arg("Cg") = 0);
  m.def("conv_set_bk", [](int64_t bk) { pva_bf16::conv_igemm_set_bk((int)bk); pva_f16::conv_igemm_set_bk((int)bk); });
  m.def("conv_set_ut", [](int64_t mode) { pva_bf16::conv_igemm_set_ut((int)mode); pva_f16::conv_igemm_set_ut((int)mode); });
  m.def("wgrad_rt_legal", [](int64_t Cout, int64_t Cin, int64_t ldd, int64_t ldx, int64_t chunk) {
    return pva_bf16::wgrad_rt_legal((int)Cout, (int)Cin, (int)ldd, (int)ldx, (int)chunk, 0) != 0;
  });
  m.def("wgrad_tile", &wgrad_tile, py::arg("Cout"), py::arg("K"), py::arg("variant") = -1);
  m.def("wgrad_narrow_legal", [](int64_t Cout, int64_t Cin, int64_t K) {
    return (bool)pva_bf16::wgrad_narrow_legal((int)Cout, (int)Cin, (int)K);
  });
  m.def("conv_wgrad", &conv_wgrad, py::arg("dy"), py::arg("x"), py::arg("partial"), py::arg("scale"),
        py::arg("shift"), py::arg("affine"), py::arg("g"), py::arg("chunk"), py::arg("slab") = 0,
        py::arg("variant") = -1, py::arg("dy_affine") = 0, py::arg("colsum") = py::none());
  m.def("wgrad_reduce", &wgrad_reduce, py::arg("partial"), py::arg("grad"), py::arg("splits"), py::arg("Cout"),
        py::arg("taps"), py::arg("Cin"), py::arg("Cin_real"), py::arg("scale"), py::arg("beta"), py::arg("slab") = 0);
  m.def("bn_finalize", &bn_finalize, py::arg("part"), py::arg("tiles"), py::arg("C"), py::arg("count"),
        py::arg("gamma"), py::arg("beta"), py::arg("rm"), py::arg("rv"), py::arg("nbt"), py::arg("momentum"),
        py::arg("eps"), py::arg("smean"), py::arg("srstd"), py::arg("scale"), py::arg("shift"),
        py::arg("fin") = py::none());
  m.def("fin_doubles", [](int64_t C) { return fin_doubles(C); });
  m.def("bn_eval_affine", &bn_eval_affine);
  m.def("bn_act", &bn_act);
  m.def("res_out", &res_out);
  m.def("bn_bwd_blocks", &bn_bwd_blocks);
  m.def("bn_bwd_reduce", &bn_bwd_reduce, py::arg("g"), py::arg("ldg"), py::arg("mask_mode"), py::arg("mo"),
        py::arg("ldm"), py::arg("ms"), py::arg("mh"), py::arg("y0"), py::arg("mean0"), py::arg("rstd0"), py::arg("y1"),
        py::arg("mean1"), py::arg("rstd1"), py::arg("M"), py::arg("C"), py::arg("blocks"), py::arg("rpb"),
        py::arg("part"), py::arg("dzout") = py::none(), py::arg("lddz") = 0);
  m.def("bn_bwd_finalize", &bn_bwd_finalize, py::arg("part"), py::arg("blocks"), py::arg("C"), py::arg("count"),
        py::arg("which"), py::arg("gamma"), py::arg("mean"), py::arg("rstd"), py::arg("dgamma"), py::arg("dbeta"),
        py::arg("beta_acc"), py::arg("coef"), py::arg("fin") = py::none());
  m.def("bn_bwd_apply", &bn_bwd_apply);
  m.def("stem_pool_fwd", &stem_pool_fwd, py::arg("y"), py::arg("scale"), py::arg("shift"), py::arg("out"),
        py::arg("ldo"), py::arg("arg"), py::arg("NT"), py::arg("H"), py::arg("W"), py::arg("Ho"), py::arg("Wo"),
        py::arg("C"), py::arg("ymax") = py::none());
  m.def("stem_pool_bn_apply", &stem_pool_bn_apply);
  m.def("stem_pool_bwd", &stem_pool_bwd);
  m.def("avgpool_fwd", &avgpool_fwd);
  m.def("avgpool_bwd", &avgpool_bwd);
  m.def("sgd_momentum", &sgd_momentum, py::arg("p"), py::arg("g"), py::arg("buf"), py::arg("lr"),
        py::arg("momentum"), py::arg("wd"), py::arg("gscale"), py::arg("first"), py::arg("found_inf"),
        py::arg("skip_if") = py::none());
  m.def("nonfinite_check", &nonfinite_check);
  m.def("pack_weights", &pack_weights);
  m.def("pack_desc_size", &pva_bf16::pack_desc_size);
  m.def("video_preprocess", &video_preprocess, py::arg("frames"), py::arg("desc"), py::arg("tidx"), py::arg("T"),
        py::arg("S"), py::arg("mean"), py::arg("std"), py::arg("out"), py::arg("s2d"), py::arg("slow_of") = py::none(),
        py::arg("slow_out") = py::none(), py::arg("Ts") = 0);
  m.def("synth_frames", &synth_frames);
  m.def("narrow_c_bwd", &narrow_c_bwd, py::arg("g"), py::arg("ldg"), py::arg("mode"), py::arg("mask"), py::arg("yc"),
        py::arg("coef"), py::arg("dz"), py::arg("lddz"), py::arg("dz_accum"), py::arg("yb"), py::arg("sb"),
        py::arg("hb"), py::arg("mb"), py::arg("rb"), py::arg("wc"), py::arg("dab"), py::arg("ldo"), py::arg("accum"),
        py::arg("slab"), py::arg("part"), py::arg("M"), py::arg("CO"), py::arg("CI"), py::arg("rps"),
        py::arg("form") = 0, py::arg("y1") = py::none(), py::arg("mc") = py::none(), py::arg("rc") = py::none(),
        py::arg("m1") = py::none(), py::arg("r1") = py::none(), py::arg("cpart") = py::none());
  m.def("lateral_bwd", &lateral_bwd);
  m.def("lateral_bwd_legal", [](int64_t CO, int64_t Cf, int64_t alpha, int64_t To, int64_t Tf, int64_t kt, int64_t pad) {
    return (bool)pva_bf16::lateral_bwd_legal((int)CO, (int)Cf, (int)alpha, (int)To, (int)Tf, (int)kt, (int)pad);
  });
  m.def("narrow_c_bwd_legal", [](int64_t CO, int64_t CI) { return (bool)pva_bf16::narrow_c_bwd_legal((int)CO, (int)CI); });
  m.def("narrow_c_bwd_rps", [](int64_t M, int64_t CO, int64_t splits) {
    return (int64_t)pva_bf16::narrow_c_bwd_rps(M, (int)CO, (int)splits);
  });
  m.def("stem_tiles", [](int64_t Ho, int64_t Wo, int64_t N) { return pva_bf16::stem_tiles((int)Ho, (int)Wo, (int)N); });
  m.def("stem_supported", [](int64_t Cout, int64_t kt) { return pva_bf16::stem_s2d_supported((int)Cout, (int)kt); });
  m.def("head_forward", &head_forward, py::arg("feat"), py::arg("W"), py::arg("b"), py::arg("p_drop"), py::arg("seed"),
        py::arg("xm"), py::arg("logits"), py::arg("seed_dev") = py::none());
  m.def("head_seed_advance", &head_seed_advance);
  m.def("head_ce", &head_ce);
  m.def("head_backward", &head_backward, py::arg("dlogits"), py::arg("xm"), py::arg("W"), py::arg("P"),
        py::arg("p_drop"), py::arg("seed"), py::arg("dW"), py::arg("db"), py::arg("beta"), py::arg("dfeat"),
        py::arg("scratch"), py::arg("seed_dev") = py::none());
  m.def("head_dropout_mask", &head_dropout_mask);
  m.def("stem_fwd", &stem_fwd);
  m.def("stem_wgrad", &stem_wgrad, py::arg("x"), py::arg("dy"), py::arg("acc"), py::arg("dims"), py::arg("Cout"),
        py::arg("kt"), py::arg("slab") = py::none());
  m.def("stem_wgrad_convert", [](const at::Tensor& acc, const at::Tensor& grad, int64_t Cout, int64_t kt, double beta) {
    pva_bf16::stem_wgrad_convert_launch(f32(acc), f32(grad), (int)Cout, (int)kt, (float)beta, cur_stream());
  });
  m.def("stem_pack", [](const at::Tensor& w, const at::Tensor& out, int64_t Cout, int64_t kt) {
    const bool h = kind16(out);
    KSEL(h, stem_pack_launch)(f32(w), bfpm(out), (int)Cout, (int)kt, cur_stream());
  });
  register_clip_reader(m);
  register_rccl(m);
  register_fp32(m);
}
```

### pytorchvideo_accelerate_amd/models/fused.py

```python
from __future__ import annotations

import math
import os
from typing import Dict, List, Optional, Sequence, Tuple

import torch
import torch.nn as nn
import torch.nn.functional as F

from ..utils.arms import arm, on
from ..ops._ext import require
from ..ops.conv import Act, ConvSpec, dgrad_phases, fwd_geometry
from . import reference as R
from ..utils.profiling import trace_range


class _Xf:
    __slots__ = ("scale", "shift", "relu")

    def __init__(self, scale, shift, relu=True):
        self.scale, self.shift, self.relu = scale, shift, relu


class FlatParams:
# ... 450 lines not shown
                part = self.eng.scratch("bnepi", ((g[0] + 127) // 128) * 3 * g[1])
                c, one = epi.c, (None if (epi.fold1 or epi.narrow_fold) else epi.one)

            yc = None if (epi is None or epi.yc is None) else epi.yc

            def run(cfg, scratch):
                C.conv_igemm_epi(dy.t, wd, tuner.scratch_like(out) if scratch else out, 1 if accum else 0, g, 8,
                                 None if res is None else res.t, 0 if res is None else res.ld,
                                 None if epi is None else epi.mask, None if yc is None else yc.t,
                                 None if yc is None else c.mean, None if yc is None else c.rstd,
                                 None if epi is None or one is None else epi.y1.t,
                                 None if epi is None or one is None else one.mean,
                                 None if epi is None or one is None else one.rstd,
                                 None if part is None else (tuner.scratch_like(part) if scratch else part),
                                 None, None, cfg)
            cfg = tuner.launch(("er", accum, res is not None, epi is not None,
                                epi is not None and one is not None) + tuple(g), g, 8, run, epi=True)
            if epi is None:
                return None
            bm = tuner.bm(cfg, g[1])
            return part, (g[0] + bm - 1) // bm
        for g in geo:
            if accum and g[28] == 0:
                continue

            def run(cfg, scratch, g=g):
                C.conv_igemm(dy.t, wd, tuner.scratch_like(out) if scratch else out, None, None, None, 0,
                             1 if accum else 0, g, 8, cfg, bias)
            tuner.launch(("d", accum, bias is not None) + tuple(g), g, 8, run, halo=not accum and bias is None,
                         direct=bias is None)
        return None

    def bn_backward(self, g: Act, y: Act, mask_mode: int, mo: Optional[Act], mxf: Optional[_Xf],
                    dz_out: Optional[Act] = None, dz_accum: bool = False, other: Optional["_ConvBN"] = None,
                    other_y: Optional[Act] = None, pre=None) -> Tuple[Act, Optional[Act]]:
        eng, C = self.eng, self.eng.C
        M, Cc = y.M, self.C
        if isinstance(mo, Act):
            mo_t, mo_ld = mo.t, mo.ld
        else:
            mo_t, mo_ld = mo, (0 if mo is None else mo.shape[1])
        if pre is not None:
            part, blocks = pre
        else:
            blocks, rpb = eng._bn_blocks(M, Cc)
            eng.mark(self.name + ".bnred")
            part = eng.scratch("bnpart", blocks * 3 * Cc)
            C.bn_bwd_reduce(g.t, g.ld, mask_mode, mo_t, mo_ld,
                            None if mxf is None else mxf.scale, None if mxf is None else mxf.shift,
                            y.t, self.mean, self.rstd,
                            None if other is None else other_y.t, None if other is None else other.mean,
                            None if other is None else other.rstd, M, Cc, blocks, rpb, part)
        fg = eng.flat
        C.bn_bwd_finalize(part, blocks, Cc, M, 0, self.bn.weight, self.mean, self.rstd,
                          fg.gview(self.bn.weight), fg.gview(self.bn.bias), eng.grad_beta, self.coef, self.fin)
        if other is not None:
            C.bn_bwd_finalize(part, blocks, Cc, M, 1, other.bn.weight, other.mean, other.rstd,
                              fg.gview(other.bn.weight), fg.gview(other.bn.bias), eng.grad_beta, other.coef,
                              other.fin)
        dy = eng.ws((self.name, "dy"), (M, Cc), eng.cdt)
        dy1 = eng.ws((other.name, "dy"), (M, Cc), eng.cdt) if other is not None else None
        eng.mark(self.name + ".bnapply")
        C.bn_bwd_apply(g.t, g.ld, mask_mode, mo_t, mo_ld,
                       None if mxf is None else mxf.scale, None if mxf is None else mxf.shift,
                       y.t, self.coef, dy, None if other is None else other_y.t,
                       None if other is None else other.coef, dy1,
                       None if dz_out is None else dz_out.t, 0 if dz_out is None else dz_out.ld,
                       1 if dz_accum else 0, M, Cc)
        a = Act(dy, y.N, y.T, y.H, y.W)
        b = Act(dy1, y.N, y.T, y.H, y.W) if other is not None else None
        return a, b


def to_s2d(x_ncthw: torch.Tensor, dtype: torch.dtype = torch.bfloat16) -> Act:
    N, C, T, H, W = x_ncthw.shape
    x = F.pad(x_ncthw, (0, 0, 0, 0, 0, 0, 0, 4 - C))
    x = x.reshape(N, 4, T, H // 2, 2, W // 2, 2).permute(0, 2, 3, 5, 4, 6, 1)
    x = x.reshape(N * T * (H // 2) * (W // 2), 16).contiguous().to(dtype)
    return Act(x, N, T, H // 2, W // 2)


class _Stem:

    def __init__(self, eng, stem: R.ResNetBasicStem, name: str):
        self.u = _ConvBN(eng, stem.conv, stem.norm, name + ".conv", cin_pad=4)
        self.eng, self.name = eng, name
        self.units = [self.u]
        k = tuple(stem.conv.kernel_size)
        self.kt = k[0]
        self.s2d = (eng.stem_s2d and k[1:] == (7, 7) and tuple(stem.conv.stride) == (1, 2, 2)
                    and tuple(stem.conv.padding) == (self.kt // 2, 3, 3) and stem.conv.in_channels == 3
                    and eng.C.stem_supported(self.u.C, self.kt))
        if self.s2d:
            cpad = (self.u.C + 15) // 16 * 16
            self.wpack = torch.zeros(cpad * self.kt * 256, device=eng.device, dtype=eng.cdt)

    def out_channels(self):
        return self.u.C

    def out_dims(self, T, H, W):
        if self.s2d:
            return T, (H - 1) // 2 + 1, (W - 1) // 2 + 1
        To, Ho, Wo = self.u.spec.out_dims(T, H, W)
        return To, (Ho - 1) // 2 + 1, (Wo - 1) // 2 + 1

    def pack(self):
        if self.s2d:
            self.eng.C.stem_pack(self.eng.flat.view(self.u.conv.weight), self.wpack, self.u.C, self.kt)

    def _conv_s2d(self, x: Act, train: bool, tag: str) -> Act:
        eng, C, u = self.eng, self.eng.C, self.u
        assert x.C == 16 and x.t.is_contiguous(), "s2d stem expects a dense [M, 16] space-to-depth input"
        M = x.M
        y = eng.ws((u.name, "y", tag), (M, u.C), eng.cdt)
        tiles = C.stem_tiles(x.H, x.W, x.N)
        stats = eng.ws((u.name, "stats"), (tiles, 2, u.C), torch.float32)
        eng.mark(u.name + ".fwd")
        C.stem_fwd(x.t, self.wpack, y, stats, [x.N, x.T, x.H, x.W], u.C, self.kt)
        bn = u.bn
        if train:
            C.bn_finalize(stats, tiles, u.C, M, bn.weight, bn.bias, bn.running_mean, bn.running_var,
                          bn.num_batches_tracked, bn.momentum if bn.momentum is not None else 0.1, bn.eps,
                          u.mean, u.rstd, u.scale, u.shift, u.fin)
        else:
            C.bn_eval_affine(bn.weight, bn.bias, bn.running_mean, bn.running_var, bn.eps, u.scale, u.shift)
        return Act(y, x.N, x.T, x.H, x.W)

    def fwd(self, x: Act, out: torch.Tensor, train: bool, tag: str) -> Act:
        C = self.eng.C
        y = self._conv_s2d(x, train, tag) if self.s2d else self.u.fwd(x, None, train, tag)
        Ho, Wo = (y.H - 1) // 2 + 1, (y.W - 1) // 2 + 1
        P = y.N * y.T * Ho * Wo
        arg = self.eng.ws((self.name, "arg"), (P, self.u.C), torch.uint8)
        ymax = self.eng.ws((self.name, "ymax"), (P, self.u.C), self.eng.cdt) if train else None
        self.eng.mark(self.name + ".pool")
        C.stem_pool_fwd(y.t, self.u.scale, self.u.shift, out, out.stride(0), arg, y.N * y.T, y.H, y.W, Ho, Wo,
                        self.u.C, ymax)
        self.x, self.y, self.arg, self.ymax = x, y, arg, ymax
        return Act(out, y.N, y.T, Ho, Wo)

    def bwd(self, dout: Act):
        eng, C, u = self.eng, self.eng.C, self.u
        y = self.y
        assert self.ymax is not None, "stem backward needs a training-mode forward"
        P = dout.M
        blocks, rpb = eng._bn_blocks(P, u.C)
        eng.mark(u.name + ".bnred")
        part = eng.scratch("bnpart", blocks * 3 * u.C)
        C.bn_bwd_reduce(dout.t, dout.ld, 2, None, 0, u.scale, u.shift, self.ymax, u.mean, u.rstd, None, None, None,
                        P, u.C, blocks, rpb, part)
        fg = eng.flat
        C.bn_bwd_finalize(part, blocks, u.C, y.M, 0, u.bn.weight, u.mean, u.rstd, fg.gview(u.bn.weight),
                          fg.gview(u.bn.bias), eng.grad_beta, u.coef, u.fin)
        dyt = eng.ws((u.name, "dy"), (y.M, u.C), eng.cdt)
        eng.mark(self.name + ".poolbwd")
        C.stem_pool_bn_apply(dout.t, dout.ld, self.arg, y.t, u.scale, u.shift, u.coef, dyt, y.N * y.T, y.H, y.W,
                             dout.H, dout.W, u.C)
        dy = Act(dyt, y.N, y.T, y.H, y.W)
        if self.s2d:
            x = self.x
            acc = eng.scratch("stem_acc_" + self.name, self.u.C * self.kt * 256, zero=True)
            eng.mark(self.u.name + ".wgrad")
            slab = None
            if eng.reproducible:
                slab = eng.scratch("stem_slab_" + self.name,
                                   C.stem_tiles(x.H, x.W, x.N) * self.u.C * self.kt * 256)
            C.stem_wgrad(x.t, dy.t, acc, [x.N, x.T, x.H, x.W], self.u.C, self.kt, slab)
            C.stem_wgrad_convert(acc, eng.flat.gview(self.u.conv.weight), self.u.C, self.kt, eng.grad_beta)
        else:
            self.u.wgrad(dy, self.x, None)


class _ResBlock:
    def __init__(self, eng, blk: R.ResBlock, name: str):
        b2 = blk.branch2
        self.eng, self.name = eng, name
        self.a = _ConvBN(eng, b2.conv_a, b2.norm_a, name + ".a")
        self.b = _ConvBN(eng, b2.conv_b, b2.norm_b, name + ".b")
        self.c = _ConvBN(eng, b2.conv_c, b2.norm_c, name + ".c")
        self.one = _ConvBN(eng, blk.branch1_conv, blk.branch1_norm, name + ".1") if blk.branch1_conv is not None else None
        self.units = [u for u in (self.a, self.b, self.c, self.one) if u is not None]
        sc = self.c.spec
        self.fold = (eng.bn_fold and tuple(sc.k) == (1, 1, 1) and tuple(sc.stride) == (1, 1, 1) and sc.cin % 8 == 0
                     and sc.cout % 8 == 0 and sc.cin >= eng.fold_min_c)
        self.narrow_c = (not self.fold and eng.narrow_bwd and tuple(sc.k) == (1, 1, 1) and tuple(sc.stride) == (1, 1, 1)
                         and sc.cin == 8 and sc.cin_pad == 8 and bool(eng.C.narrow_c_bwd_legal(sc.cout, sc.cin)))
        self.narrow_fold = self.narrow_c and eng.narrow_fold
        s1 = self.one.spec if self.one is not None else None
        self.fold1 = (self.fold and s1 is not None and eng.bn_fold1 and tuple(s1.k) == (1, 1, 1)
                      and tuple(s1.stride) == (1, 1, 1) and s1.cin % 8 == 0 and s1.cin == s1.cin_pad
                      and s1.cin <= 2048)

    def out_channels(self):
        return self.c.C

    def out_dims(self, T, H, W):
        return self.b.spec.out_dims(T, H, W)

    def fwd(self, x: Act, out: torch.Tensor, train: bool, tag: str) -> Act:
        C = self.eng.C
        ya = self.a.fwd(x, None, train, tag)
        yb = self.b.fwd(ya, self.a.xf(), train, tag)
        if self.fold:
            y1 = self.one.fwd(x, None, train, tag) if self.one is not None else None
            if self.fold1 and train:
                self.one.fold_branch1_forward(x)
            self.c.fold_forward(yb, self.b.xf(), train)
            mask = self.eng.ws((self.name, "mask", tag), (yb.M, self.c.C // 8), torch.uint8)
            res, rxf = (x, None) if y1 is None else (y1, self.one.xf(relu=False))
            o = self.c.fold_output(yb, self.b.xf(), out, res, rxf, mask, tag)
            self.mask = mask if train else None
            self.x, self.ya, self.yb, self.yc, self.y1, self.out = x, ya, yb, None, y1, o
            return o
        if self.narrow_fold:
            y1 = self.one.fwd(x, None, train, tag) if self.one is not None else None
            self.c.narrow_fold_stats(yb, self.b.xf(), train)
            mask = self.eng.ws((self.name, "mask", tag), (yb.M, self.c.C // 8), torch.uint8)
            res, rxf = (x, None) if y1 is None else (y1, self.one.xf(relu=False))
            o = self.c.fold_output(yb, self.b.xf(), out, res, rxf, mask, tag)
            self.mask = mask if train else None
            self.x, self.ya, self.yb, self.yc, self.y1, self.out = x, ya, yb, None, y1, o
            return o
        yc = self.c.fwd(yb, self.b.xf(), train, tag)
        y1 = self.one.fwd(x, None, train, tag) if self.one is not None else None
        M = yc.M
        self.eng.mark(self.name + ".res_out")
        mask = self.eng.ws((self.name, "mask"), (M, self.c.C // 8), torch.uint8) if train else None
        C.res_out(yc.t, self.c.scale, self.c.shift,
                  None if y1 is None else y1.t, None if y1 is None else self.one.scale,
                  None if y1 is None else self.one.shift, None if y1 is not None else x.t, x.ld,
                  out, out.stride(0), M, self.c.C, mask)
        self.mask = mask
        o = Act(out, yc.N, yc.T, yc.H, yc.W)
        self.x, self.ya, self.yb, self.yc, self.y1, self.out = x, ya, yb, yc, y1, o
        return o

    def bwd(self, dout: Act, dx: torch.Tensor, dx_accum: bool, pre=None, prev: Optional["_ResBlock"] = None):
        eng = self.eng
        x, ya, yb, yc, y1 = self.x, self.ya, self.yb, self.yc, self.y1
        dxa = Act(dx, x.N, x.T, x.H, x.W)
        res = None
        if self.fold:
            return self._bwd_fold(dout, dx, dx_accum, pre, prev)
        if self.narrow_c:
            return self._bwd_narrow(dout, dx, dx_accum, pre, prev)
        if pre is not None:
            dyc, dy1 = self.c.bn_backward(dout, yc, 0, None, None, other=self.one, other_y=y1, pre=pre)
            if self.one is None:
                res = dout
        elif self.one is None:
            dyc, _ = self.c.bn_backward(dout, yc, 3, self.mask, None, dz_out=dxa, dz_accum=dx_accum)
        else:
            dyc, dy1 = self.c.bn_backward(dout, yc, 3, self.mask, None, other=self.one, other_y=y1)
        self.c.wgrad(dyc, yb, self.b.xf())
        dab = eng.ws((self.name, "dab"), (yb.M, self.b.C), eng.cdt)
        pb = self.c.dgrad(dyc, (yb.T, yb.H, yb.W), dab, False, bn=(self.b, yb))
        dyb, _ = self.b.bn_backward(Act(dab, yb.N, yb.T, yb.H, yb.W), yb, 0 if pb else 2, None,
                                    None if pb else self.b.xf(), pre=pb)
        self.b.wgrad(dyb, ya, self.a.xf())
        daa = eng.ws((self.name, "daa"), (ya.M, self.a.C), eng.cdt)
        pa = self.b.dgrad(dyb, (ya.T, ya.H, ya.W), daa, False, bn=(self.a, ya))
        dya, _ = self.a.bn_backward(Act(daa, ya.N, ya.T, ya.H, ya.W), ya, 0 if pa else 2, None,
                                    None if pa else self.a.xf(), pre=pa)
        self.a.wgrad(dya, x, None)
        if self.one is not None:
            self.one.wgrad(dy1, x, None)
            if self._strided_one(prev):
                return self._dgrad_strided_one(dya, dy1, dx, dx_accum)
            self.one.dgrad(dy1, (x.T, x.H, x.W), dx, dx_accum)
            acc = True
        else:
            acc = dx_accum if pre is not None else True
        if prev is not None and not self._epi_ok(prev):
            prev = None
        if res is None and prev is None:
            self.a.dgrad(dya, (x.T, x.H, x.W), dx, acc)
            return None
        return self.a.dgrad(dya, (x.T, x.H, x.W), dx, acc, res=res, epi=prev)

    def _bwd_narrow(self, dout: Act, dx: torch.Tensor, dx_accum: bool, pre, prev: Optional["_ResBlock"]):
        eng, C = self.eng, self.eng.C
        x, ya, yb, yc, y1, one, c = self.x, self.ya, self.yb, self.yc, self.y1, self.one, self.c
        dxa = Act(dx, x.N, x.T, x.H, x.W)
        M, Cc = yb.M, c.C
        fg = eng.flat
        res = None
        rps = int(C.narrow_c_bwd_rps(M, Cc, eng.narrow_splits))
        splits = (M + rps - 1) // rps
        b = self.b
        if self.narrow_fold:
            if pre is not None:
                mode, mask, dz_out = 0, None, None
                if one is None:
                    res = dout
            else:
                mode, mask = 3, self.mask
                dz_out = dxa if one is None else None
            part = eng.scratch("narrow_cpart", splits * 3 * Cc)
            blocks = splits
            eng.mark(c.name + ".foldred")
            C.narrow_c_bwd(dout.t, dout.ld, mode, mask, None, c.coef, None, 0, 0, yb.t, b.scale, b.shift, b.mean,
                           b.rstd, c.wf, None, 8, 0, None, None, M, Cc, yb.C, rps, form=2,
                           y1=None if one is None else y1.t, mc=c.mean, rc=c.rstd,
                           m1=None if one is None else one.mean, r1=None if one is None else one.rstd, cpart=part)
        elif pre is not None:
            part, blocks = pre
# ... 144 lines not shown

    def _dgrad_strided_one(self, dya: Act, dy1: Act, dx: torch.Tensor, dx_accum: bool):
        x = self.x
        self.a.dgrad(dya, (x.T, x.H, x.W), dx, dx_accum)
        self.one.dgrad(dy1, (x.T, x.H, x.W), dx, True)
        return None

    def _epi_ok(self, prev: "_ResBlock") -> bool:
        s = self.a.spec
        return (tuple(s.stride) == (1, 1, 1) and prev.out.t.is_contiguous() and prev.c.C % 8 == 0
                and prev.mask is not None)


class _Stage:
    def __init__(self, eng, stage: R.ResStage, name: str):
        self.blocks = [_ResBlock(eng, b, f"{name}.{i}") for i, b in enumerate(stage.res_blocks)]
        self.eng, self.name = eng, name
        self.units = [u for b in self.blocks for u in b.units]

    def out_channels(self):
        return self.blocks[-1].out_channels()

    def out_dims(self, T, H, W):
        for b in self.blocks:
            T, H, W = b.out_dims(T, H, W)
        return T, H, W

    def fwd(self, x: Act, out: torch.Tensor, train: bool, tag: str) -> Act:
        eng = self.eng
        for i, b in enumerate(self.blocks):
            if i == len(self.blocks) - 1:
                o = out
            else:
                T, H, W = b.out_dims(x.T, x.H, x.W)
                o = eng.ws((b.name, "out", tag), (x.N * T * H * W, b.out_channels()), eng.cdt)
            x = b.fwd(x, o, train, tag)
        return x

    def bwd(self, dout: Act, dx: torch.Tensor, dx_accum: bool):
        eng = self.eng
        pre = None
        for i in range(len(self.blocks) - 1, -1, -1):
            b = self.blocks[i]
            if i == 0:
                tgt, acc = dx, dx_accum
            else:
                xin = b.x
                tgt, acc = eng.ws((b.name, "dx"), (xin.M, xin.C), eng.cdt), False
            pre = b.bwd(dout, tgt, acc, pre=pre, prev=self.blocks[i - 1] if i > 0 else None)
            b.eng_progress(b.flat_hi)
            if i > 0:
                xin = b.x
                dout = Act(tgt, xin.N, xin.T, xin.H, xin.W)


class _Fuse:
    def __init__(self, eng, f: R.FuseFastToSlow, name: str):
        self.u = _ConvBN(eng, f.conv_fast_to_slow, f.norm, name)
        self.eng, self.name = eng, name
        self.units = [self.u]
        self.lateral_used = False

    def fwd(self, xf: Act, cat_slice: torch.Tensor, train: bool, tag: str):
        y = self.u.fwd(xf, None, train, tag)
        self.eng.mark(self.name + ".bn_act")
        self.eng.C.bn_act(y.t, y.ld, cat_slice, cat_slice.stride(0), self.u.scale, self.u.shift, 1, y.M, self.u.C)
        self.xf_in, self.y = xf, y

    def _lateral_ok(self, x: Act, dcat_slice: Act, dfast: torch.Tensor) -> bool:
        s, y = self.u.spec, self.y
        return (self.eng.lateral_bwd and tuple(s.k[1:]) == (1, 1) and tuple(s.stride[1:]) == (1, 1)
                and tuple(s.pad[1:]) == (0, 0) and s.cin_pad == s.cin and (y.H, y.W) == (x.H, x.W)
                and dcat_slice.ld % 8 == 0 and dfast.stride(0) % 8 == 0
                and bool(self.eng.C.lateral_bwd_legal(s.cout, s.cin, s.stride[0], y.T, x.T, s.k[0], s.pad[0])))

    def bwd(self, dcat_slice: Act, dfast: torch.Tensor):
        y, u, eng = self.y, self.u, self.eng
        x = self.xf_in
        self.lateral_used = self._lateral_ok(x, dcat_slice, dfast)
        if self.lateral_used:
            C = eng.C
            M, Cc = y.M, u.C
            blocks, rpb = eng._bn_blocks(M, Cc)
            eng.mark(u.name + ".bnred")
            part = eng.scratch("bnpart", blocks * 3 * Cc)
            C.bn_bwd_reduce(dcat_slice.t, dcat_slice.ld, 2, None, 0, u.scale, u.shift, y.t, u.mean, u.rstd,
                            None, None, None, M, Cc, blocks, rpb, part)
            fg = eng.flat
            C.bn_bwd_finalize(part, blocks, Cc, M, 0, u.bn.weight, u.mean, u.rstd, fg.gview(u.bn.weight),
                              fg.gview(u.bn.bias), eng.grad_beta, u.coef, u.fin)
            dy = eng.ws((u.name, "dy"), (M, Cc), eng.cdt)
            eng.mark(self.name + ".latbwd")
            C.lateral_bwd(dcat_slice.t, dcat_slice.ld, y.t, u.scale, u.shift, u.coef, u.wd, dy, dfast,
                          dfast.stride(0), x.N, y.T, x.T, y.H * y.W, Cc, u.spec.cin, u.spec.stride[0])
            u.wgrad(Act(dy, y.N, y.T, y.H, y.W), x, None)
            return
        dy, _ = u.bn_backward(dcat_slice, y, 2, None, u.xf())
        u.wgrad(dy, x, None)
        u.dgrad(dy, (x.T, x.H, x.W), dfast, True)


class FusedNet:

    def __init__(self, model: R.Net, device: torch.device, stem_s2d: bool = True, deterministic: bool = False,
                 load_tuning: bool = True, compute_dtype: torch.dtype = torch.bfloat16, reproducible: bool = False):
        assert compute_dtype in (torch.bfloat16, torch.float16), compute_dtype
        self.cdt = compute_dtype
        self.C = require()
        self.deterministic = deterministic
        self.reproducible = reproducible
        self.fold_slabs = deterministic or reproducible or on("fold_slabs")
        self.lateral_bwd = on("lateral_bwd")
        self.side_fuse = on("side_fuse")
        self.stem_s2d = stem_s2d and not deterministic
        self.model = model
        self.device = torch.device(device)
        model.to(self.device)
        self.prof: Optional[List] = None
        from ..ops.tune import ConvTuner
        self.tuner = ConvTuner(require(), enabled=not deterministic and torch.device(device).type == "cuda")
        self.wtune: Dict = {}
        self._eval_tune: Dict = {}
        from ..ops.tune import TuneStore
        self.tune_store = None
        if self.tuner.enabled:
            self.tune_store = TuneStore({"conv": self.tuner.cache, "eval": self._eval_tune, "wgrad": self.wtune},
                                        TuneStore.build_ident(self.device, str(compute_dtype)))
            if load_tuning:
                self.tune_store.load()
        self._ws: Dict = {}
        self._splits: Dict = {}
        self._bnb: Dict = {}
        self._scratch: Dict[Tuple, torch.Tensor] = {}
        self._fin: Dict[int, torch.Tensor] = {}
        self._cmax = 8
        self.grad_beta = 0.0
        self.lane = 0
        self._side = None
        self._seed_dev = None
        self._ms_warm = False
        self._ms_bwd = False
        self._wst = [None, None]
        self._wst_used = [False, False]
        self.debug_skip_joins = set()
        self._ms_ok = (not deterministic and torch.device(device).type == "cuda"
                       and on("streams"))
        self.bn_fold = on("bn_fold")
        self.fold_min_c = int(arm("bn_fold_min_c"))
        self.bn_fold1 = self.bn_fold and on("bn_fold1")
        self.fold_exact_below = int(arm("bn_fold_exact_below"))
        self.narrow_bwd = on("narrow_bwd")
        self.narrow_splits = int(arm("narrow_splits"))
        self.narrow_fold = self.narrow_bwd and on("narrow_fold")
        blocks = list(model.blocks)
        self.slowfast = isinstance(blocks[0], R.MultiPathWayWithFuse)
        self.stages: List[Tuple[List, Optional[_Fuse]]] = []
        if self.slowfast:
            for i, b in enumerate(blocks):
                if not isinstance(b, R.MultiPathWayWithFuse):
                    break
                paths = []
                for p, m in enumerate(b.multipathway_blocks):
                    nm = f"b{i}.p{p}"
                    paths.append(_Stem(self, m, nm) if isinstance(m, R.ResNetBasicStem) else _Stage(self, m, nm))
                fuse = _Fuse(self, b.multipathway_fusion, f"b{i}.fuse") if b.multipathway_fusion is not None else None
                self.stages.append((paths, fuse))
            pool = blocks[-2]
            assert isinstance(pool, R.PoolConcatPathway)
            self.head_pools = [tuple(p.kernel_size) for p in pool.pool]
            self.head = blocks[-1]
        else:
            for i, b in enumerate(blocks[:-1]):
                nm = f"b{i}.p0"
                self.stages.append(([_Stem(self, b, nm) if isinstance(b, R.ResNetBasicStem) else _Stage(self, b, nm)],
                                    None))
            self.head = blocks[-1]
            self.head_pools = [tuple(self.head.pool.kernel_size)] if self.head.pool is not None else [None]
        self.npath = len(self.stages[0][0])
        self.units: List[_ConvBN] = []
        for paths, fuse in self.stages:
            for p in paths:
                self.units += p.units
            if fuse is not None:
                self.units += fuse.units
        self._cmax = max(u.C for u in self.units)
        order = list(self.head.named_parameters(prefix="head"))
        for u in reversed(self.units):
            order += [(u.name + ".bn.w", u.bn.weight), (u.name + ".bn.b", u.bn.bias), (u.name + ".w", u.conv.weight)]
        seen = set()
        named = []
        for n, p in order:
            if id(p) not in seen:
                seen.add(id(p))
                named.append((n, p))
        assert len(named) == len(list(model.parameters())), "executor does not cover every parameter"
        self.flat = FlatParams(named, self.device)
        self._build_packs()
        self.pack()
        self.grad_hook = None
        self.grad_multi_stream = False
        self._head_hi = max(self.flat.span(p)[1] for p in self.head.parameters())
        for paths, fuse in self.stages:
            mods = list(paths) + ([fuse] if fuse is not None else [])
            for m in mods:
                subs = m.blocks if isinstance(m, _Stage) else [m]
                for sub in subs:
                    sub.flat_hi = max(self.flat.span(w)[1] for u in sub.units
                                      for w in (u.conv.weight, u.bn.weight, u.bn.bias))
                    sub.eng_progress = self._progress

    def mark(self, label: str):
        if self.prof is not None:
            ev = torch.cuda.Event(enable_timing=True)
            ev.record()
            self.prof.append((label, ev))

    def profile_report(self) -> List[Tuple[str, float]]:
        torch.cuda.synchronize()
        p = self.prof or []
        return [(a, e0.elapsed_time(e1)) for (a, e0), (_, e1) in zip(p, p[1:])]

    def producer_streams(self) -> List:
        out = [torch.cuda.current_stream(self.device)]
        if self._side is not None:
            out.append(self._side)
        out += [st for st in self._wst if st is not None]
        return out

    def _progress(self, hi: int, force: bool = False):
        if self.grad_hook is not None and self.grad_multi_stream:
            self.grad_hook(hi)
            return
        if self.grad_hook is not None and (force or not self._ms_bwd):
            if force:
                self._join_wgrads()
            self.grad_hook(hi)

    def ws(self, key, shape, dtype) -> torch.Tensor:
        t = self._ws.get(key)
        if t is None or tuple(t.shape) != tuple(shape) or t.dtype != dtype:
            t = torch.empty(shape, device=self.device, dtype=dtype)
            self._ws[key] = t
        return t

    def fin_ws(self) -> Optional[torch.Tensor]:
        if self.device.type != "cuda":
            return None
        t = self._fin.get(self.lane)
        if t is None:
            t = self._fin[self.lane] = torch.zeros(self.C.fin_doubles(self._cmax), device=self.device,
                                                   dtype=torch.float64)
        return t

    def scratch(self, key: str, numel: int, zero: bool = False) -> torch.Tensor:
        k = (key, self.lane)
        t = self._scratch.get(k)
        if t is None or t.numel() < numel:
            alloc = torch.zeros if zero else torch.empty
            t = alloc(max(numel, 1 << 20), device=self.device, dtype=torch.float32)
            self._scratch[k] = t
        return t[:numel]

    def _ms_active(self) -> bool:
        return (self._ms_ok and self._ms_warm and self.npath == 2 and self.prof is None)

    def _side_stream(self):
        if self._side is None:
            self._side = torch.cuda.Stream(device=self.device,
                                           priority=int(arm("side_priority")))
        return self._side

    def _wgrad_stream(self):
        i = self.lane
        if self._wst[i] is None:
            self._wst[i] = torch.cuda.Stream(device=self.device)
        self._wst_used[i] = True
        return self._wst[i]

    def _join_wgrads(self):
        main = torch.cuda.current_stream(self.device)
        for i, st in enumerate(self._wst):
            if st is not None and self._wst_used[i]:
                self._join(main, st)
                self._wst_used[i] = False

    def _join(self, waiter, signaller, tag: Optional[str] = None):
        if tag is not None and tag in self.debug_skip_joins:
            return
        ev = torch.cuda.Event()
        ev.record(signaller)
        waiter.wait_event(ev)

    def _bn_blocks(self, M, C):
        k = (M, C)
        v = self._bnb.get(k)
        if v is None:
            v = self._bnb[k] = tuple(self.C.bn_bwd_blocks(M, C))
        return v

    def _build_packs(self):
        fwd_n, dgr_n = 0, 0
        offs = []
        for u in self.units:
            s = u.spec
            nf = s.cout * s.taps * s.cin_pad
            nd = s.cin * s.taps * s.cout if s.cin % 8 == 0 else 0
# ... 259 lines not shown
```

### pytorchvideo_accelerate_amd/utils/arms.py

```python
from __future__ import annotations

import os
from typing import Dict, Optional, Union

Value = Union[int, str, None]

DEFAULTS: Dict[str, tuple] = {
    "autotune": (1, "r1: heuristic configs only when 0"),
    "conv_direct": (1, "r3_knobs"),
    "conv_dma": (1, "r3_knobs"),
    "conv_pw": (1, "r2_final"),
    "conv_halo": (1, "r3_halo"),
    "conv_halo_d": (1, "r6_halo: double-buffered 64-channel halo conv as a tuner candidate"),
    "conv_big_half": (1, "r4_big_half"),
    "conv_pf": (1, "r5_lab"),
    "conv_pw_w4": (1, "r5_lateral"),
    "pw_kinds": (None, "debugging aid: restrict the pointwise kernel to these launch kinds"),
    "tune_reps": (3, "r4_tune_reps"),
    "tune_top": (3, "r4_tune_reps"),
    "streams": (1, "r2_final: two-stream execution"),
    "side_priority": (0, "r5_hwq"),
    "side_fuse": (1, "r5_side"),
    "lateral_bwd": (1, "r5_lateral"),
    "fold_slabs": (1, "r4_regress"),
    "bn_fold": (1, "r2_pmc_final"),
    "bn_fold_min_c": (16, "r4_fold"),
    "bn_fold1": (1, "r3_fold1"),
    "bn_fold_exact_below": (32, "r4_fold (scripts/diag_ms_fold.py @ a59cdac)"),
    "narrow_bwd": (1, "r5_narrow"),
    "narrow_splits": (1024, "r5_narrow"),
    "narrow_fold": (1, "r5_narrow"),
    "f32_pieces": (3, "r6_f32"),
    "stem_pair": (1, "r4_stem"),
    "stem_perm": (1, "r5_end"),
    "stem_roll": (1, "r5_stem_roll"),
    "stem_async": (1, "r5_stem_roll"),
}


def _parse(spec: str) -> Dict[str, str]:
    out = {}
    for item in spec.split(","):
        item = item.strip()
        if not item:
            continue
        if "=" not in item:
            raise ValueError(f"PVA_ARMS entry {item!r} is not name=value")
        k, v = item.split("=", 1)
        k = k.strip()
        if k not in DEFAULTS:
            raise ValueError(f"PVA_ARMS: unknown arm {k!r} (known: {', '.join(sorted(DEFAULTS))})")
        out[k] = v.strip()
    return out


def arm(name: str) -> Value:
    dflt = DEFAULTS[name][0]
    v = _parse(os.environ.get("PVA_ARMS", "")).get(name)
    if v is None:
        return dflt
    if isinstance(dflt, int):
        return int(v)
    return v


def on(name: str) -> bool:
    return bool(arm(name))


def arms_spec(**kw) -> str:
    cur = _parse(os.environ.get("PVA_ARMS", ""))
    for k, v in kw.items():
        if k not in DEFAULTS:
            raise ValueError(f"unknown arm {k!r}")
        cur[k] = str(int(v) if isinstance(v, bool) else v)
    return ",".join(f"{k}={v}" for k, v in cur.items())


def selected() -> Dict[str, Optional[Value]]:
    return {k: arm(k) for k in DEFAULTS if arm(k) != DEFAULTS[k][0]}
```

### pytorchvideo_accelerate_amd/utils/depcheck.py

```python
from __future__ import annotations

import contextlib
import re
from dataclasses import dataclass
from typing import Dict, List, Optional, Tuple

import torch

WRITES: Dict[str, Tuple[str, ...]] = {
    "conv_igemm": ("y", "stats"),
    "conv_igemm_epi": ("y", "part"),
    "conv_igemm_fres": ("y", "mask"),
    "conv_wgrad": ("partial", "colsum"),
    "wgrad_reduce": ("partial", "grad"),
    "wgrad_box_reduce": ("tmp", "grad"),
    "bn_finalize": ("rm", "rv", "nbt", "smean", "srstd", "scale", "shift", "fin"),
    "bn_eval_affine": ("scale", "shift"),
    "bn_act": ("out",),
    "res_out": ("out", "mask"),
    "bn_bwd_reduce": ("part", "dzout"),
    "bn_bwd_finalize": ("dgamma", "dbeta", "coef", "fin"),
    "bn_bwd_apply": ("dy0", "dy1", "dzout"),
    "stem_pool_fwd": ("out", "arg", "ymax"),
    "stem_pool_bn_apply": ("dy",),
    "stem_pool_bwd": ("dact",),
    "avgpool_fwd": ("out",),
    "avgpool_bwd": ("dx",),
    "pack_weights": ("fwd", "dgr"),
    "stem_fwd": ("y", "stats"),
    "stem_wgrad": ("acc", "slab"),
    "stem_wgrad_convert": ("acc", "grad"),
    "stem_pack": ("out",),
    "bnfold_fwd_stats": ("T", "s_out", "rm", "rv", "nbt", "smean", "srstd", "scale", "shift"),
    "bnfold_bwd": ("dgamma", "dbeta", "dW", "coef", "W1t", "W2", "bias"),
    "head_forward": ("xm", "logits"),
    "head_seed_advance": ("seed_dev",),
    "head_ce": ("dlogits", "loss", "counts", "row_loss", "row_correct"),
    "head_backward": ("dW", "db", "dfeat", "scratch"),
    "head_dropout_mask": ("out",),
    "lateral_bwd": ("dy", "dx"),
    "narrow_c_bwd": ("dz", "dab", "slab", "part", "cpart"),
    "nonfinite_check": ("flag",),
    "sgd_momentum": ("p", "buf", "found_inf"),
    "video_preprocess": ("out", "slow_out"),
}

ARGNAMES: Dict[str, Tuple[str, ...]] = {
    "avgpool_bwd": ("dout", "ldo", "coff", "dims", "k", "dx"),
    "avgpool_fwd": ("x", "dims", "k", "out", "ldo", "coff"),
    "bn_act": ("y", "ldy", "out", "ldo", "scale", "shift", "relu", "M", "C"),
    "bn_bwd_apply": ("g", "ldg", "mask_mode", "mo", "ldm", "ms", "mh", "y0", "coef0", "dy0", "y1", "coef1", "dy1",
                     "dzout", "lddz", "dz_accum", "M", "C"),
    "bn_eval_affine": ("gamma", "beta", "rm", "rv", "eps", "scale", "shift"),
    "bnfold_bwd": ("part", "tiles", "Wf", "Wd", "G", "T", "s", "C", "c", "count", "gamma", "mean", "rstd", "dgamma",
                   "dbeta", "dW", "beta_acc", "coef", "W1t", "W2", "bias"),
    "bnfold_fwd_stats": ("Wf", "Ga", "sslab", "splits", "C", "c", "count", "T", "s_out", "gamma", "beta", "rm", "rv",
                         "nbt", "momentum", "eps", "smean", "srstd", "scale", "shift"),
    "conv_igemm_fres": ("x", "w", "y", "scale", "shift", "affine", "g", "chunk", "cfg", "osc", "osh", "res", "ldr",
                        "rsc", "rsh", "mask"),
    "head_ce": ("logits", "labels", "gscale", "dlogits", "loss", "counts", "acc_counts", "row_loss", "row_correct"),
    "head_dropout_mask": ("out", "p_drop", "seed"),
    "head_seed_advance": ("seed_dev",),
    "lateral_bwd": ("g", "ldg", "y", "sc", "sh", "coef", "wd", "dy", "dx", "ldx", "N", "To", "Tf", "HW", "CO", "Cf",
                    "alpha"),
    "nonfinite_check": ("g", "gscale", "flag"),
    "pack_weights": ("master", "fwd", "dgr", "descs", "ntensors"),
    "res_out": ("yc", "sc", "hc", "y1", "s1", "h1", "x", "ldx", "out", "ldo", "M", "C", "mask"),
    "stem_fwd": ("x", "wpack", "y", "stats", "dims", "Cout", "kt"),
    "stem_pack": ("w", "out", "Cout", "kt"),
    "stem_pool_bn_apply": ("dout", "ldd", "arg", "y", "ms", "mh", "coef", "dy", "NT", "H", "W", "Ho", "Wo", "C"),
    "stem_pool_bwd": ("dout", "ldd", "arg", "dact", "NT", "H", "W", "Ho", "Wo", "C"),
    "stem_wgrad_convert": ("acc", "grad", "Cout", "kt", "beta"),
    "wgrad_box_reduce": ("slab", "tmp", "grad", "splits", "Cout", "taps", "Cin", "Cin_real", "scale", "beta"),
}


@dataclass
class Hazard:
    kind: str
    fn: str
    arg: str
    stream: int
    count: int
    other_fn: str
    other_stream: int
    other_count: int

    def __str__(self):
        return (f"{self.kind}: {self.fn}({self.arg}) on stream {self.stream:#x} #{self.count} vs {self.other_fn} on "
                f"stream {self.other_stream:#x} #{self.other_count} without a wait")


def _arg_names(fn, name: str) -> Optional[Tuple[str, ...]]:
    if name in ARGNAMES:
        return ARGNAMES[name]
    doc = (getattr(fn, "__doc__", "") or "").split("\n")[0]
    if "(" not in doc:
        return None
    inner = doc[doc.index("(") + 1:doc.rindex(")")]
    names = tuple(re.findall(r"(?:^|,\s*)(\w+):", inner))
    return None if any(n.startswith("arg") and n[3:].isdigit() for n in names) else names


def _span(t: torch.Tensor) -> Tuple[int, int, int]:
    base = t.untyped_storage().data_ptr()
    lo = t.data_ptr()
    if t.numel() == 0:
        return base, lo, lo
    ext = 1 + sum((s - 1) * st for s, st in zip(t.shape, t.stride()) if s > 0)
    return base, lo, lo + ext * t.element_size()


class DepChecker:
    def __init__(self, raise_on_hazard: bool = False):
        self.raise_on_hazard = raise_on_hazard
        self.count: Dict[int, int] = {}
        self.clock: Dict[int, Dict[int, int]] = {}
        self.events: Dict[int, Dict[int, int]] = {}
        self.acc: Dict[int, Dict[Tuple[int, int, str, int], Tuple[int, str]]] = {}
        self.hazards: List[Hazard] = []
        self.launches = 0
        self._names: Dict[str, Optional[Tuple[str, ...]]] = {}

    @staticmethod
    def _sid(stream=None) -> int:
        s = stream if stream is not None else torch.cuda.current_stream()
        return int(s.cuda_stream)

    def on_record(self, event, stream=None):
        s = self._sid(stream)
        snap = dict(self.clock.get(s, {}))
        snap[s] = self.count.get(s, 0)
        self.events[id(event)] = snap

    def on_wait(self, stream, event):
        snap = self.events.get(id(event))
        if snap is None:
            return
        c = self.clock.setdefault(self._sid(stream), {})
        for k, v in snap.items():
            if c.get(k, 0) < v:
                c[k] = v

    def on_sync(self):
        everything = dict(self.count)
        for s in set(self.count) | set(self.clock):
            c = self.clock.setdefault(s, {})
            for k, v in everything.items():
                if c.get(k, 0) < v:
                    c[k] = v

    def on_launch(self, name: str, fn, args, kwargs):
        names = self._names.get(name, False)
        if names is False:
            names = self._names[name] = _arg_names(fn, name)
        writes = set(WRITES.get(name, ()))
        tensors = []
        for i, a in enumerate(args):
            if isinstance(a, torch.Tensor) and a.is_cuda:
                nm = names[i] if names is not None and i < len(names) else f"arg{i}"
                tensors.append((nm, a))
        for k, a in kwargs.items():
            if isinstance(a, torch.Tensor) and a.is_cuda:
                tensors.append((k, a))
        s = self._sid()
        cnt = self.count.get(s, 0) + 1
        self.count[s] = cnt
        self.launches += 1
        seen = self.clock.setdefault(s, {})
        for nm, t in tensors:
            w = nm in writes or (names is None and name not in WRITES)
            base, lo, hi = _span(t)
            if hi <= lo:
                continue
            recs = self.acc.setdefault(base, {})
            for (rlo, rhi, kind, rs), (rc, rfn) in recs.items():
                if rs == s or rhi <= lo or rlo >= hi:
                    continue
                if kind == "w" or w:
                    if seen.get(rs, 0) < rc:
                        hz = Hazard(("WAW" if w else "RAW") if kind == "w" else "WAR", name, nm, s, cnt, rfn, rs, rc)
                        self.hazards.append(hz)
                        if self.raise_on_hazard:
                            raise RuntimeError(str(hz))
            key_r = (lo, hi, "r", s)
            recs[key_r] = (cnt, name)
            if w:
                recs[(lo, hi, "w", s)] = (cnt, name)

    @contextlib.contextmanager
    def watching(self):
        ev_record = torch.cuda.Event.record
        st_wait = torch.cuda.Stream.wait_event
        dev_sync = torch.cuda.synchronize
        ev_sync = torch.cuda.Event.synchronize
        chk = self

        def record(ev, stream=None):
            chk.on_record(ev, stream)
            return ev_record(ev, stream) if stream is not None else ev_record(ev)

        def wait_event(st, ev):
            chk.on_wait(st, ev)
            return st_wait(st, ev)

        def synchronize(device=None):
            chk.on_sync()
            return dev_sync(device)

        def ev_synchronize(ev):
            chk.on_sync()
            return ev_sync(ev)

        torch.cuda.Event.record = record
        torch.cuda.Stream.wait_event = wait_event
        torch.cuda.synchronize = synchronize
        torch.cuda.Event.synchronize = ev_synchronize
        try:
            yield self
        finally:
            torch.cuda.Event.record = ev_record
            torch.cuda.Stream.wait_event = st_wait
            torch.cuda.synchronize = dev_sync
            torch.cuda.Event.synchronize = ev_sync

# ... 41 lines not shown
```

Before: 494.5 clips/s.

## Fuse stem maxpool/BN backward into stem weight-gradient kernel

Adds a fused variant of the stem wgrad kernels that computes the pool-backward plus BN-apply dy on the fly from pooled gradients, argmax indices and saved activations. The results are staged into the LDS dy tile, replacing the separate stem_pool_bn_apply kernel and its dy buffer round trip through global memory. Loads for the next time step are issued early and finished after the MFMA loop to overlap latency. It costs extra registers and LDS in the wgrad kernel, which may lower occupancy. The path is controlled by a new arm flag that defaults to on.

```diff
diff --git a/csrc/kernels/bn_eltwise.hip b/csrc/kernels/bn_eltwise.hip
--- a/csrc/kernels/bn_eltwise.hip
+++ b/csrc/kernels/bn_eltwise.hip
@@ -559,20 +559,9 @@
 #pragma unroll
           for (int j = 0; j <= b; ++j) {
             const uint32_t want = (uint32_t)((i ? 0 : a + 1) * 3 + (j ? 0 : b + 1));
-            const uint2 pk = ag[i][j];
-#pragma unroll
-            for (int e = 0; e < 8; ++e) {
-              const uint32_t bi = ((e < 4 ? pk.x : pk.y) >> (8 * (e & 3))) & 255u;
-              acc[e] += bi == want ? g[i][j][e] : 0.f;
-            }
+            stem_dz_gather(acc, ag[i][j], g[i][j], want);
           }
-        float o8[8];
-#pragma unroll
-        for (int e = 0; e < 8; ++e) {
-          const float dz = (yv[e] * MS[e] + MH[e]) > 0.f ? acc[e] : 0.f;
-          o8[e] = A[e] * dz + B[e] * yv[e] + Cc[e];
-        }
-        *reinterpret_cast<uint4*>(dy + m * C + c) = pack8(o8);
+        *reinterpret_cast<uint4*>(dy + m * C + c) = stem_dy_chunk(yv, acc, A, B, Cc, MS, MH);
       }
     }
   }
diff --git a/csrc/kernels/common.h b/csrc/kernels/common.h
--- a/csrc/kernels/common.h
+++ b/csrc/kernels/common.h
@@ -88,6 +88,25 @@
   return make_uint2(pack2(f[0], f[1]), pack2(f[2], f[3]));
 }
 
+__device__ __forceinline__ void stem_dz_gather(float* acc, const uint2 pk, const float* g, uint32_t want) {
+#pragma unroll
+  for (int e = 0; e < 8; ++e) {
+    const uint32_t bi = ((e < 4 ? pk.x : pk.y) >> (8 * (e & 3))) & 255u;
+    acc[e] += bi == want ? g[e] : 0.f;
+  }
+}
+
+__device__ __forceinline__ uint4 stem_dy_chunk(const float* yv, const float* acc, const float* A, const float* B,
+                                               const float* Cc, const float* MS, const float* MH) {
+  float o8[8];
+#pragma unroll
+  for (int e = 0; e < 8; ++e) {
+    const float dz = (yv[e] * MS[e] + MH[e]) > 0.f ? acc[e] : 0.f;
+    o8[e] = A[e] * dz + B[e] * yv[e] + Cc[e];
+  }
+  return pack8(o8);
+}
+
 __device__ __forceinline__ int xcd_remap(int orig, int nwg) {
   if (nwg < PVA_NXCD * 2) return orig;
   const int q = nwg / PVA_NXCD, r = nwg % PVA_NXCD;
diff --git a/csrc/kernels/launchers.h b/csrc/kernels/launchers.h
--- a/csrc/kernels/launchers.h
+++ b/csrc/kernels/launchers.h
@@ -68,6 +68,9 @@
 int stem_tiles(int Ho, int Wo, int N);
 void stem_s2d_launch(int mode, const uint16_t* x, const uint16_t* w, uint16_t* y, float* stats, const uint16_t* dy,
                      float* dw, int N, int T, int Hs, int Ws, int Cout, int kt, hipStream_t s, float* slab = nullptr);
+void stem_s2d_fused_bwd_launch(const uint16_t* x, const uint16_t* dout, int ldd, const uint8_t* arg, const uint16_t* y,
+                               const float* scale, const float* shift, const float* coef, float* dw, int N, int T,
+                               int Hs, int Ws, int Cout, int kt, int Hp, int Wp, hipStream_t s, float* slab = nullptr);
 bool stem_s2d_supported(int Cout, int kt);
 void stem_wgrad_convert_launch(float* acc, float* grad, int Cout, int kt, float beta, hipStream_t s);
 void stem_pack_launch(const float* w, uint16_t* out, int Cout, int kt, hipStream_t s);
diff --git a/csrc/kernels/stem_s2d.hip b/csrc/kernels/stem_s2d.hip
--- a/csrc/kernels/stem_s2d.hip
+++ b/csrc/kernels/stem_s2d.hip
@@ -23,6 +23,12 @@
   int pt;
   int tiles_h, tiles_w;
   int slab;
+  const uint16_t* dout;
+  const uint8_t* arg;
+  const float* scale;
+  const float* shift;
+  const float* coef;
+  int ldd, Hp, Wp;
 };
 
 constexpr uint32_t OOB = 0x7ffffff0u;
@@ -201,7 +207,37 @@
   return __builtin_bit_cast(ev8_t, v);
 }
 
-template <int KT, int COT, bool AR = false>
+typedef __attribute__((ext_vector_type(4))) uint32_t u32x4_t;
+typedef __attribute__((ext_vector_type(2))) uint32_t u32x2_t;
+
+__device__ __forceinline__ u32x4_t ld16(__amdgpu_buffer_rsrc_t r, uint32_t vo) {
+  return __builtin_bit_cast(u32x4_t, __builtin_amdgcn_raw_buffer_load_b128(r, (int)vo, 0, 0));
+}
+__device__ __forceinline__ u32x2_t ld8(__amdgpu_buffer_rsrc_t r, uint32_t vo) {
+  return __builtin_bit_cast(u32x2_t, __builtin_amdgcn_raw_buffer_load_b64(r, (int)vo, 0, 0));
+}
+__device__ __forceinline__ void vm_hold(u32x4_t& v) { asm volatile("" : "+v"(v)); }
+__device__ __forceinline__ void vm_hold(u32x2_t& v) { asm volatile("" : "+v"(v)); }
+
+__device__ __forceinline__ void fuse_dz(float* acc, const u32x4_t (&g0)[2], const u32x2_t (&a0)[2],
+                                        const u32x4_t (&g1)[2], const u32x2_t (&a1)[2], int pa, int pb) {
+#pragma unroll
+  for (int e = 0; e < 8; ++e) acc[e] = 0.f;
+#pragma unroll
+  for (int i = 0; i < 2; ++i)
+#pragma unroll
+    for (int j = 0; j < 2; ++j) {
+      if (i > pa || j > pb) continue;
+      const uint32_t want = (uint32_t)((i ? 0 : pa + 1) * 3 + (j ? 0 : pb + 1));
+      const u32x4_t g = i ? g1[j] : g0[j];
+      const u32x2_t a = i ? a1[j] : a0[j];
+      float gf[8];
+      unpack8(__builtin_bit_cast(uint4, g), gf);
+      stem_dz_gather(acc, make_uint2(a[0], a[1]), gf, want);
+    }
+}
+
+template <int KT, int COT, bool AR = false, bool FU = false>
 __global__ __launch_bounds__(256) void stem_wgrad_kernel(const StemParams p) {
   constexpr int TAPS = KT * 16;
   constexpr int TPW = TAPS / 4;
@@ -222,7 +258,7 @@
   const int ho0 = th * TH, wo0 = tw * TW;
   const __amdgpu_buffer_rsrc_t xr =
       clip_rsrc(p.x + (int64_t)n * p.T * p.Hs * p.Ws * 16, (uint32_t)(p.T * p.Hs * p.Ws * 32));
-  const __amdgpu_buffer_rsrc_t yr = clip_rsrc(p.dy + (int64_t)n * p.To * p.Ho * p.Wo * p.Cout,
+  const __amdgpu_buffer_rsrc_t yr = clip_rsrc((FU ? p.y : p.dy) + (int64_t)n * p.To * p.Ho * p.Wo * p.Cout,
                                               (uint32_t)(p.To * p.Ho * p.Wo * p.Cout * 2));
   auto dma_dy = [&](int to, char* buf) {
 #pragma unroll
@@ -235,6 +271,73 @@
       dma16(yr, buf + (k * 256 + w * 64) * 16, vo);
     }
   };
+  static_assert(!FU || DYC == 1 || (DYC == 4 && COP == 64), "fused staging: one position or a 2x2 block per lane");
+  constexpr int CPP = COP / 8;
+  const int fch = (tid % CPP) * 8, fblk = tid / CPP;
+  const int fr0 = DYC == 4 ? 2 * (fblk / (TW / 2)) : fblk / TW, fc0 = DYC == 4 ? 2 * (fblk % (TW / 2)) : fblk % TW;
+  const int fho = ho0 + fr0, fwo = wo0 + fc0;
+  const int hp0 = fho >> 1, wp0 = fwo >> 1;
+  float* cf = reinterpret_cast<float*>(dyt + 2 * DYB);
+  const int64_t pq = (int64_t)n * p.To * p.Hp * p.Wp;
+  const __amdgpu_buffer_rsrc_t dr =
+      clip_rsrc(FU ? p.dout + pq * p.ldd : nullptr, FU ? (uint32_t)(((p.To * p.Hp * p.Wp - 1) * p.ldd + p.Cout) * 2) : 0u);
+  const __amdgpu_buffer_rsrc_t ar =
+      clip_rsrc(FU ? reinterpret_cast<const uint16_t*>(p.arg + pq * p.Cout) : nullptr,
+                FU ? (uint32_t)(p.To * p.Hp * p.Wp * p.Cout) : 0u);
+  u32x4_t fy[DYC], fg[2][2];
+  u32x2_t fa[2][2];
+  auto fuse_issue = [&](int to) {
+#pragma unroll
+    for (int k = 0; k < DYC; ++k) {
+      const int ho = fho + (k >> 1), wo = fwo + (k & 1);
+      const bool ok = ho < p.Ho && wo < p.Wo && fch < p.Cout;
+      fy[k] = ld16(yr, ok ? (uint32_t)((((to * p.Ho + ho) * p.Wo + wo) * p.Cout + fch) * 2) : OOB);
+    }
+#pragma unroll
+    for (int i = 0; i < 2; ++i)
+#pragma unroll
+      for (int j = 0; j < 2; ++j) {
+        const int hp = hp0 + i, wp = wp0 + j;
+        const bool need = DYC == 4 || ((i == 0 || (fho & 1)) && (j == 0 || (fwo & 1)));
+        const bool ok = need && fho < p.Ho && fwo < p.Wo && hp < p.Hp && wp < p.Wp && fch < p.Cout;
+        const int q = (to * p.Hp + hp) * p.Wp + wp;
+        fg[i][j] = ld16(dr, ok ? (uint32_t)((q * p.ldd + fch) * 2) : OOB);
+        fa[i][j] = ld8(ar, ok ? (uint32_t)(q * p.Cout + fch) : OOB);
+      }
+  };
+  auto fuse_finish = [&](char* buf) {
+#pragma unroll
+    for (int k = 0; k < DYC; ++k) vm_hold(fy[k]);
+#pragma unroll
+    for (int i = 0; i < 2; ++i)
+#pragma unroll
+      for (int j = 0; j < 2; ++j) { vm_hold(fg[i][j]); vm_hold(fa[i][j]); }
+    float K[5][8];
+#pragma unroll
+    for (int i = 0; i < 5; ++i)
+#pragma unroll
+      for (int e = 0; e < 8; e += 4)
+        *reinterpret_cast<float4*>(&K[i][e]) = *reinterpret_cast<const float4*>(cf + i * COP + fch + e);
+#pragma unroll
+    for (int k = 0; k < DYC; ++k) {
+      const int ho = fho + (k >> 1), wo = fwo + (k & 1);
+      const bool ok = ho < p.Ho && wo < p.Wo && fch < p.Cout;
+      float yv[8], acc[8];
+      unpack8(__builtin_bit_cast(uint4, fy[k]), yv);
+      fuse_dz(acc, fg[0], fa[0], fg[1], fa[1], DYC == 4 ? k >> 1 : ho & 1, DYC == 4 ? k & 1 : wo & 1);
+      const uint4 v = stem_dy_chunk(yv, acc, K[0], K[1], K[2], K[3], K[4]);
+      const int pos = (fr0 + (k >> 1)) * TW + fc0 + (k & 1);
+      *reinterpret_cast<uint4*>(buf + (pos * CPP + tid % CPP) * 16) = ok ? v : make_uint4(0, 0, 0, 0);
+    }
+  };
+  if constexpr (FU) {
+    for (int i = tid; i < 5 * COP; i += 256) {
+      const int c = i % COP, m = i / COP;
+      const float* src = m < 3 ? p.coef + m * p.Cout : (m == 3 ? p.scale : p.shift);
+      cf[i] = c < p.Cout ? src[c] : 0.f;
+    }
+    __syncthreads();
+  }
 
   f32x4_t acc[COT][TPW];
 #pragma unroll
@@ -243,14 +346,16 @@
     for (int t = 0; t < TPW; ++t) acc[c][t] = f32x4_t{0.f, 0.f, 0.f, 0.f};
 
   for (int f = 0; f < KT; ++f) dma_patch(xr, p, f - p.pt, ho0, wo0, smem + f * SLOT_BYTES);
-  dma_dy(0, dyt);
+  if constexpr (FU) { fuse_issue(0); fuse_finish(dyt); }
+  else dma_dy(0, dyt);
   __syncthreads();
   const int rq = li >> 2, cb = (li & 3) * 8;
   for (int to = 0; to < p.To; ++to) {
     const char* dcur = dyt + (to & 1) * DYB;
     if (to + 1 < p.To) {
       dma_patch(xr, p, to - p.pt + KT, ho0, wo0, smem + ((to + KT) % SLOTS) * SLOT_BYTES);
-      dma_dy(to + 1, dyt + ((to + 1) & 1) * DYB);
+      if constexpr (FU) fuse_issue(to + 1);
+      else dma_dy(to + 1, dyt + ((to + 1) & 1) * DYB);
     }
     if constexpr (AR) {
       constexpr int KS = TH * TW / 32, NR = COT + TPW;
@@ -292,6 +397,7 @@
           for (int c = 0; c < COT; ++c) acc[c][t] = PVA_MFMA16(frag8(Rk[c][0], Rk[c][1]), xb, acc[c][t], 0, 0, 0);
         }
       }
+      if (FU && to + 1 < p.To) fuse_finish(dyt + ((to + 1) & 1) * DYB);
       __syncthreads();
       continue;
     }
@@ -321,6 +427,7 @@
           acc[c][t] = PVA_MFMA16(a[c], xb, acc[c][t], 0, 0, 0);
       }
     }
+    if (FU && to + 1 < p.To) fuse_finish(dyt + ((to + 1) & 1) * DYB);
     __syncthreads();
   }
 #pragma unroll
@@ -440,7 +547,7 @@
   }
 }
 
-template <int KT, bool ROLL, bool AR = false>
+template <int KT, bool ROLL, bool AR = false, bool FU = false>
 __global__ __launch_bounds__(256) __attribute__((amdgpu_waves_per_eu(2))) void stem_wgrad_pair_kernel(const StemParams p) {
   constexpr int TAPS = KT * 16;
   constexpr int J = KT + 1;
@@ -460,7 +567,7 @@
   const __amdgpu_buffer_rsrc_t xr =
       clip_rsrc(p.x + (int64_t)n * p.T * p.Hs * p.Ws * 16, (uint32_t)(p.T * p.Hs * p.Ws * 32));
   const __amdgpu_buffer_rsrc_t yr =
-      clip_rsrc(p.dy + (int64_t)n * p.To * p.Ho * p.Wo * 8, (uint32_t)(p.To * p.Ho * p.Wo * 16));
+      clip_rsrc((FU ? p.y : p.dy) + (int64_t)n * p.To * p.Ho * p.Wo * 8, (uint32_t)(p.To * p.Ho * p.Wo * 16));
   const int dpos = pswz(tid >> 1), dfh = tid & 1;
   const int dho = ho0 + dpos / TW, dwo = wo0 + dpos % TW;
   const bool dok = dho < p.Ho && dwo < p.Wo;
@@ -469,6 +576,55 @@
     const uint32_t vo = dok && to < p.To ? (uint32_t)((((to * p.Ho + dho) * p.Wo + dwo) * 8) * 2) : OOB;
     dma16(yr, buf + w * 64 * 16, vo);
   };
+  const int64_t pq = (int64_t)n * p.To * p.Hp * p.Wp;
+  const __amdgpu_buffer_rsrc_t dr =
+      clip_rsrc(FU ? p.dout + pq * p.ldd : nullptr, FU ? (uint32_t)(((p.To * p.Hp * p.Wp - 1) * p.ldd + 8) * 2) : 0u);
+  const __amdgpu_buffer_rsrc_t ar =
+      clip_rsrc(FU ? reinterpret_cast<const uint16_t*>(p.arg + pq * 8) : nullptr,
+                FU ? (uint32_t)(p.To * p.Hp * p.Wp * 8) : 0u);
+  float K[5][8];
+  if constexpr (FU) {
+#pragma unroll
+    for (int e = 0; e < 8; ++e) {
+      K[0][e] = p.coef[e]; K[1][e] = p.coef[8 + e]; K[2][e] = p.coef[16 + e];
+      K[3][e] = p.scale[e]; K[4][e] = p.shift[e];
+    }
+  }
+  const int fdf = lane & 1, fc = (lane >> 1) & 7, fr = lane >> 4;
+  u32x4_t fy, fg[2][2];
+  u32x2_t fa[2][2];
+  auto fuse_class = [&](int t0) { return __builtin_amdgcn_readfirstlane((w + (t0 >> 1)) & 3); };
+  auto fuse_issue = [&](int t0) {
+    const int cls = fuse_class(t0), pa = cls >> 1, pb = cls & 1;
+    const int ho = ho0 + 2 * fr + pa, wo = wo0 + 2 * fc + pb, to = t0 + fdf;
+    const bool okc = ho < p.Ho && wo < p.Wo && to < p.To;
+    fy = ld16(yr, okc ? (uint32_t)((((to * p.Ho + ho) * p.Wo + wo) * 8) * 2) : OOB);
+#pragma unroll
+    for (int i = 0; i < 2; ++i)
+#pragma unroll
+      for (int j = 0; j < 2; ++j) {
+        const int hp = (ho >> 1) + i, wp = (wo >> 1) + j;
+        const bool ok = okc && i <= pa && j <= pb && hp < p.Hp && wp < p.Wp;
+        const int q = (to * p.Hp + hp) * p.Wp + wp;
+        fg[i][j] = ld16(dr, ok ? (uint32_t)(q * p.ldd * 2) : OOB);
+        fa[i][j] = ld8(ar, ok ? (uint32_t)(q * 8) : OOB);
+      }
+  };
+  auto fuse_finish = [&](int t0, char* buf) {
+    vm_hold(fy);
+#pragma unroll
+    for (int i = 0; i < 2; ++i)
+#pragma unroll
+      for (int j = 0; j < 2; ++j) { vm_hold(fg[i][j]); vm_hold(fa[i][j]); }
+    const int cls = fuse_class(t0), pa = cls >> 1, pb = cls & 1;
+    const int row = 2 * fr + pa, col = 2 * fc + pb;
+    const bool okc = ho0 + row < p.Ho && wo0 + col < p.Wo && t0 + fdf < p.To;
+    float yv[8], acc[8];
+    unpack8(__builtin_bit_cast(uint4, fy), yv);
+    fuse_dz(acc, fg[0], fa[0], fg[1], fa[1], pa, pb);
+    const uint4 v = stem_dy_chunk(yv, acc, K[0], K[1], K[2], K[3], K[4]);
+    *reinterpret_cast<uint4*>(buf + (pswz(row * TW + col) * 2 + fdf) * 16) = okc ? v : make_uint4(0, 0, 0, 0);
+  };
 
   f32x4_t acc[J][4];
 #pragma unroll
@@ -477,7 +633,8 @@
     for (int s = 0; s < 4; ++s) acc[j][s] = f32x4_t{0.f, 0.f, 0.f, 0.f};
 
   for (int f = 0; f < J; ++f) dma_patch<true>(xr, p, f - p.pt, ho0, wo0, smem + f * SLOT_BYTES);
-  dma_dy(0, dyt);
+  if constexpr (FU) { fuse_issue(0); fuse_finish(0, dyt); }
+  else dma_dy(0, dyt);
   __syncthreads();
   const int rq = li >> 2, cb = (li & 3) * 8;
   for (int t0 = 0; t0 < p.To; t0 += 2) {
@@ -486,8 +643,13 @@
       const int tn = t0 - p.pt + J;
       dma_patch<true>(xr, p, tn, ho0, wo0, smem + ((t0 + J) % SLOTS) * SLOT_BYTES);
       dma_patch<true>(xr, p, tn + 1, ho0, wo0, smem + ((t0 + J + 1) % SLOTS) * SLOT_BYTES);
-      dma_dy(t0 + 2, dyt + (((t0 >> 1) + 1) & 1) * DYB);
-    }
+      if constexpr (FU) fuse_issue(t0 + 2);
+      else dma_dy(t0 + 2, dyt + (((t0 >> 1) + 1) & 1) * DYB);
+    }
+    auto fuse_next = [&]() {
+      if constexpr (FU)
+        if (t0 + 2 < p.To) fuse_finish(t0 + 2, dyt + (((t0 >> 1) + 1) & 1) * DYB);
+    };
     if constexpr (ROLL && AR) {
       constexpr int KS = TH * TW / 32;
       const int h0 = g >> 1, wq = 8 * (g & 1) + rq;
@@ -534,6 +696,7 @@
           acc[j][3] = PVA_MFMA16(af[kstep], frag8(F[kstep + 1][2], F[kstep + 1][3]), acc[j][3], 0, 0, 0);
         }
       }
+      fuse_next();
       __syncthreads();
       continue;
     }
@@ -570,6 +733,7 @@
           fo = fo2;
         }
       }
+      fuse_next();
       __syncthreads();
       continue;
     }
@@ -596,6 +760,7 @@
         }
       }
     }
+    fuse_next();
     __syncthreads();
   }
 #pragma unroll
@@ -666,10 +831,10 @@
   hipLaunchKernelGGL((stem_fwd_kernel<KT, COT, PERM>), dim3(p.N * p.tiles_h * p.tiles_w), dim3(256), lds, s, p);
 }
 
-template <int KT, int COT, bool AR = false>
+template <int KT, int COT, bool AR = false, bool FU = false>
 void launch_wgrad(const StemParams& p, hipStream_t s) {
-  const size_t lds = (KT + 1) * SLOT_BYTES + 2 * TH * TW * COT * 16 * 2;
-  hipLaunchKernelGGL((stem_wgrad_kernel<KT, COT, AR>), dim3(p.N * p.tiles_h * p.tiles_w), dim3(256), lds, s, p);
+  const size_t lds = (KT + 1) * SLOT_BYTES + 2 * TH * TW * COT * 16 * 2 + (FU ? 5 * COT * 16 * 4 : 0);
+  hipLaunchKernelGGL((stem_wgrad_kernel<KT, COT, AR, FU>), dim3(p.N * p.tiles_h * p.tiles_w), dim3(256), lds, s, p);
 }
 
 template <int KT>
@@ -678,10 +843,10 @@
   hipLaunchKernelGGL((stem_fwd_pair_kernel<KT>), dim3(p.N * p.tiles_h * p.tiles_w), dim3(256), lds, s, p);
 }
 
-template <int KT, bool ROLL, bool AR = false>
+template <int KT, bool ROLL, bool AR = false, bool FU = false>
 void launch_wgrad_pair(const StemParams& p, hipStream_t s) {
   const size_t lds = (KT + 3) * SLOT_BYTES + 2 * TH * TW * 16 * 2;
-  hipLaunchKernelGGL((stem_wgrad_pair_kernel<KT, ROLL, AR>), dim3(p.N * p.tiles_h * p.tiles_w), dim3(256), lds, s, p);
+  hipLaunchKernelGGL((stem_wgrad_pair_kernel<KT, ROLL, AR, FU>), dim3(p.N * p.tiles_h * p.tiles_w), dim3(256), lds, s, p);
 }
 
 }
@@ -702,6 +867,18 @@
 static bool stem_perm_enabled() { return stem_arm("stem_perm") != 0; }
 static bool stem_roll_enabled() { return stem_arm("stem_roll") != 0; }
 static bool stem_async_enabled() { return stem_arm("stem_async") != 0; }
+
+template <bool FU>
+static void wgrad_select(const StemParams& p, int kt, hipStream_t s) {
+  const int Cout = p.Cout;
+  const bool pair = stem_pair_enabled() && kt == 5 && Cout == 8;
+  if (pair && stem_roll_enabled() && stem_async_enabled()) launch_wgrad_pair<5, true, true, FU>(p, s);
+  else if (pair && stem_roll_enabled()) launch_wgrad_pair<5, true, false, FU>(p, s);
+  else if (pair) launch_wgrad_pair<5, false, false, FU>(p, s);
+  else if (kt == 5 && Cout <= 16) launch_wgrad<5, 1, false, FU>(p, s);
+  else if (kt == 1 && Cout <= 64 && stem_async_enabled()) launch_wgrad<1, 4, true, FU>(p, s);
+  else if (kt == 1 && Cout <= 64) launch_wgrad<1, 4, false, FU>(p, s);
+}
 
 void stem_s2d_launch(int mode, const uint16_t* x, const uint16_t* w, uint16_t* y, float* stats, const uint16_t* dy,
                      float* dw, int N, int T, int Hs, int Ws, int Cout, int kt, hipStream_t s, float* slab) {
@@ -718,16 +895,28 @@
     else if (kt == 1 && Cout == 64 && stem_perm_enabled()) launch_fwd<1, 4, true>(p, s);
     else if (kt == 1 && Cout <= 64) launch_fwd<1, 4>(p, s);
   } else {
-    if (pair && stem_roll_enabled() && stem_async_enabled()) launch_wgrad_pair<5, true, true>(p, s);
-    else if (pair && stem_roll_enabled()) launch_wgrad_pair<5, true>(p, s);
-    else if (pair) launch_wgrad_pair<5, false>(p, s);
-    else if (kt == 5 && Cout <= 16) launch_wgrad<5, 1>(p, s);
-    else if (kt == 1 && Cout <= 64 && stem_async_enabled()) launch_wgrad<1, 4, true>(p, s);
-    else if (kt == 1 && Cout <= 64) launch_wgrad<1, 4>(p, s);
+    wgrad_select<false>(p, kt, s);
     if (slab != nullptr) {
       const int n = Cout * kt * 256, nslab = p.N * p.tiles_h * p.tiles_w;
       hipLaunchKernelGGL(stem_slab_reduce_kernel, dim3((n + 255) / 256), dim3(256), 0, s, slab, nslab, n, dw);
     }
+  }
+}
+
+void stem_s2d_fused_bwd_launch(const uint16_t* x, const uint16_t* dout, int ldd, const uint8_t* arg, const uint16_t* y,
+                               const float* scale, const float* shift, const float* coef, float* dw, int N, int T,
+                               int Hs, int Ws, int Cout, int kt, int Hp, int Wp, hipStream_t s, float* slab) {
+  StemParams p{};
+  p.x = x; p.y = const_cast<uint16_t*>(y); p.dw = slab != nullptr ? slab : dw;
+  p.slab = slab != nullptr ? Cout * kt * 256 : 0;
+  p.N = N; p.T = T; p.Hs = Hs; p.Ws = Ws; p.Cout = Cout;
+  p.To = T; p.Ho = Hs; p.Wo = Ws; p.pt = kt / 2;
+  p.tiles_h = (Hs + TH - 1) / TH; p.tiles_w = (Ws + TW - 1) / TW;
+  p.dout = dout; p.ldd = ldd; p.arg = arg; p.scale = scale; p.shift = shift; p.coef = coef; p.Hp = Hp; p.Wp = Wp;
+  wgrad_select<true>(p, kt, s);
+  if (slab != nullptr) {
+    const int n = Cout * kt * 256, nslab = p.N * p.tiles_h * p.tiles_w;
+    hipLaunchKernelGGL(stem_slab_reduce_kernel, dim3((n + 255) / 256), dim3(256), 0, s, slab, nslab, n, dw);
   }
 }
 
diff --git a/csrc/runtime/bindings.cpp b/csrc/runtime/bindings.cpp
--- a/csrc/runtime/bindings.cpp
+++ b/csrc/runtime/bindings.cpp
@@ -461,6 +461,35 @@
               "stem slab too small");
   KSEL(h, stem_s2d_launch)(1, bfp(x), nullptr, nullptr, nullptr, bfp(dy), f32(acc), N, T, Hs, Ws, (int)Cout, (int)kt,
                   cur_stream(), f32o(slab));
+}
+
+void stem_wgrad_fused(const at::Tensor& x, const at::Tensor& dout, int64_t ldd, const at::Tensor& arg,
+                      const at::Tensor& y, const at::Tensor& ms, const at::Tensor& mh, const at::Tensor& coef,
+                      const at::Tensor& acc, std::vector<int64_t> dims, int64_t Cout, int64_t kt, int64_t Hp, int64_t Wp,
+                      const OptT& slab) {
+  const bool h = kind16(x);
+  TORCH_CHECK(kind16(dout) == h && kind16(y) == h, "stem fused bwd: x, dout and y must share the 16-bit type");
+  TORCH_CHECK(KSEL(h, stem_s2d_supported)((int)Cout, (int)kt), "unsupported stem");
+  TORCH_CHECK(acc.numel() >= Cout * kt * 256, "accumulator too small");
+  const int64_t N = dims[0], T = dims[1], Hs = dims[2], Ws = dims[3];
+  const int64_t P = N * T * Hp * Wp;
+  TORCH_CHECK(Cout % 8 == 0 && ldd % 8 == 0 && ldd >= Cout, "stem fused bwd: channel layout");
+  TORCH_CHECK(Hp == (Hs - 1) / 2 + 1 && Wp == (Ws - 1) / 2 + 1, "stem fused bwd: 3x3/s2/p1 pooled dims");
+  TORCH_CHECK(N * T * Hs * Ws < ((int64_t)1 << 31), "stem fused bwd: position count exceeds int32");
+  TORCH_CHECK(T * Hs * Ws * Cout * 2 <= 0x7ffffff0LL && T * Hp * Wp * ldd * 2 <= 0x7ffffff0LL,
+              "stem fused bwd: clip exceeds the 2 GiB buffer range");
+  TORCH_CHECK(x.size(1) == 16 && x.is_contiguous() && x.numel() >= N * T * Hs * Ws * 16,
+              "stem input must be dense s2d [M,16]");
+  TORCH_CHECK(y.numel() >= N * T * Hs * Ws * Cout && y.is_contiguous(), "stem fused bwd: y too small");
+  TORCH_CHECK(arg.scalar_type() == at::kByte && arg.numel() >= P * Cout && dout.dim() == 2 && dout.size(0) >= P &&
+              dout.size(1) >= Cout && dout.stride(0) == ldd && dout.stride(1) == 1,
+              "stem fused bwd: pooled buffers / row stride");
+  TORCH_CHECK(ms.numel() >= Cout && mh.numel() >= Cout && coef.numel() >= 3 * Cout, "stem fused bwd: coefficients");
+  TORCH_CHECK(!slab.has_value() || slab->numel() >= (int64_t)KSEL(h, stem_tiles)((int)Hs, (int)Ws, (int)N) * Cout * kt * 256,
+              "stem slab too small");
+  KSEL(h, stem_s2d_fused_bwd_launch)(bfp(x), bfp(dout), (int)ldd, arg.data_ptr<uint8_t>(), bfp(y), f32(ms), f32(mh),
+                                     f32(coef), f32(acc), (int)N, (int)T, (int)Hs, (int)Ws, (int)Cout, (int)kt, (int)Hp,
+                                     (int)Wp, cur_stream(), f32o(slab));
 }
 
 inline const uint64_t* seed_ptr(const OptT& t) {
@@ -756,6 +785,9 @@
   m.def("stem_fwd", &stem_fwd);
   m.def("stem_wgrad", &stem_wgrad, py::arg("x"), py::arg("dy"), py::arg("acc"), py::arg("dims"), py::arg("Cout"),
         py::arg("kt"), py::arg("slab") = py::none());
+  m.def("stem_wgrad_fused", &stem_wgrad_fused, py::arg("x"), py::arg("dout"), py::arg("ldd"), py::arg("arg"),
+        py::arg("y"), py::arg("ms"), py::arg("mh"), py::arg("coef"), py::arg("acc"), py::arg("dims"), py::arg("Cout"),
+        py::arg("kt"), py::arg("Hp"), py::arg("Wp"), py::arg("slab") = py::none());
   m.def("stem_wgrad_convert", [](const at::Tensor& acc, const at::Tensor& grad, int64_t Cout, int64_t kt, double beta) {
     pva_bf16::stem_wgrad_convert_launch(f32(acc), f32(grad), (int)Cout, (int)kt, (float)beta, cur_stream());
   });
diff --git a/pytorchvideo_accelerate_amd/models/fused.py b/pytorchvideo_accelerate_amd/models/fused.py
--- a/pytorchvideo_accelerate_amd/models/fused.py
+++ b/pytorchvideo_accelerate_amd/models/fused.py
@@ -626,6 +626,17 @@
         fg = eng.flat
         C.bn_bwd_finalize(part, blocks, u.C, y.M, 0, u.bn.weight, u.mean, u.rstd, fg.gview(u.bn.weight),
                           fg.gview(u.bn.bias), eng.grad_beta, u.coef, u.fin)
+        if self.s2d and eng.stem_fuse_bwd:
+            x = self.x
+            acc = eng.scratch("stem_acc_" + self.name, u.C * self.kt * 256, zero=True)
+            eng.mark(u.name + ".wgrad")
+            slab = None
+            if eng.reproducible:
+                slab = eng.scratch("stem_slab_" + self.name, C.stem_tiles(x.H, x.W, x.N) * u.C * self.kt * 256)
+            C.stem_wgrad_fused(x.t, dout.t, dout.ld, self.arg, y.t, u.scale, u.shift, u.coef, acc,
+                               [x.N, x.T, x.H, x.W], u.C, self.kt, dout.H, dout.W, slab)
+            C.stem_wgrad_convert(acc, fg.gview(u.conv.weight), u.C, self.kt, eng.grad_beta)
+            return
         dyt = eng.ws((u.name, "dy"), (y.M, u.C), eng.cdt)
         eng.mark(self.name + ".poolbwd")
         C.stem_pool_bn_apply(dout.t, dout.ld, self.arg, y.t, u.scale, u.shift, u.coef, dyt, y.N * y.T, y.H, y.W,
@@ -1076,6 +1087,7 @@
         self.narrow_bwd = on("narrow_bwd")
         self.narrow_splits = int(arm("narrow_splits"))
         self.narrow_fold = self.narrow_bwd and on("narrow_fold")
+        self.stem_fuse_bwd = on("stem_fuse_bwd")
         blocks = list(model.blocks)
         self.slowfast = isinstance(blocks[0], R.MultiPathWayWithFuse)
         self.stages: List[Tuple[List, Optional[_Fuse]]] = []
diff --git a/pytorchvideo_accelerate_amd/utils/arms.py b/pytorchvideo_accelerate_amd/utils/arms.py
--- a/pytorchvideo_accelerate_amd/utils/arms.py
+++ b/pytorchvideo_accelerate_amd/utils/arms.py
@@ -35,6 +35,7 @@
     "stem_perm": (1, "r5_end"),
     "stem_roll": (1, "r5_stem_roll"),
     "stem_async": (1, "r5_stem_roll"),
+    "stem_fuse_bwd": (1, "stem_fuse_bwd"),
 }
 
 
diff --git a/pytorchvideo_accelerate_amd/utils/depcheck.py b/pytorchvideo_accelerate_amd/utils/depcheck.py
--- a/pytorchvideo_accelerate_amd/utils/depcheck.py
+++ b/pytorchvideo_accelerate_amd/utils/depcheck.py
@@ -29,6 +29,7 @@
     "pack_weights": ("fwd", "dgr"),
     "stem_fwd": ("y", "stats"),
     "stem_wgrad": ("acc", "slab"),
+    "stem_wgrad_fused": ("acc", "slab"),
     "stem_wgrad_convert": ("acc", "grad"),
     "stem_pack": ("out",),
     "bnfold_fwd_stats": ("T", "s_out", "rm", "rv", "nbt", "smean", "srstd", "scale", "shift"),
@@ -71,6 +72,8 @@
     "stem_pool_bn_apply": ("dout", "ldd", "arg", "y", "ms", "mh", "coef", "dy", "NT", "H", "W", "Ho", "Wo", "C"),
     "stem_pool_bwd": ("dout", "ldd", "arg", "dact", "NT", "H", "W", "Ho", "Wo", "C"),
     "stem_wgrad_convert": ("acc", "grad", "Cout", "kt", "beta"),
+    "stem_wgrad_fused": ("x", "dout", "ldd", "arg", "y", "ms", "mh", "coef", "acc", "dims", "Cout", "kt", "Hp", "Wp",
+                         "slab"),
     "wgrad_box_reduce": ("slab", "tmp", "grad", "splits", "Cout", "taps", "Cin", "Cin_real", "scale", "beta"),
 }
 
```

Result: no change. 494.0 clips/s (-0.1%).
